# Alan-404/Conformer

Hardware: AMD Instinct MI355X
Metric: encoder audio-frames/sec (B=32,T=1000,d=512,L=16) (higher is better)
Workload: dtype f32; 1 GPU; cfg2 Conformer-L Encoder.forward: B=32/GPU, T=1000 mel frames (T'=249), d=512, 16 blocks, 8 heads, k=31, fp32, eval, random-init weights, batch-sharded replicas; per_gpu_batch=32, mel_frames=1000

## Files before the change

### conformer_amd/_lib.py

```python
from __future__ import annotations

import ctypes
import os
from ctypes import c_char_p, c_float, c_int, c_int64, c_uint64, c_void_p

_HERE = os.path.dirname(os.path.abspath(__file__))
LIB_PATH = os.environ.get("CONFORMER_AMD_LIB") or os.path.join(_HERE, "lib", "libconformer_hip.so")

_P, _I, _L, _F, _U = c_void_p, c_int, c_int64, c_float, c_uint64
ABI_VERSION = 4

SIGNATURES = {
    "cfm_version": (c_int, []),
    "cfm_abi_version": (c_int, []),
    "cfm_gemm_bias_stats_f32": (c_int, [_P, _P, _P, _P, _P, _L, _I, _I, _L, _L, _P]),
    "cfm_gemm_bias_residual_stats_f32": (c_int, [_P, _P, _P, _P, _F, _P, _P, _L, _I, _I, _L, _L, _L, _P]),
    "cfm_gemm_splitk_f32": (c_int, [_I, _P, _P, _P, _P, _F, _P, _P, _I, _L, _I, _I, _L, _L, _L, _P]),
    "cfm_gemm_lnfold_f32": (c_int, [_I, _P, _P, _I, _F, _P, _P, _P, _P, _L, _I, _I, _L, _L, _P]),
    "cfm_layernorm_fwd_stats_f32": (c_int, [_P, _P, _P, _P, _P, _L, _I, _F, _P]),
    "cfm_ffn_pack_elems": (ctypes.c_int64, [_I, _I]),
    "cfm_ffn_pack_f32": (c_int, [_P, _P, _P, _I, _I, _P]),
    "cfm_rowgemm_pack_f32": (c_int, [_P, _P, _I, _I, _I, _P]),
    "cfm_rowchain_f32": (c_int, [_I, _I, _I, _I, _P, _L, _P, _P, _P, _L, _P, _L, _P, _I, _F, _P, _P, _P, _P, _F, _I, _P, _L, _P, _P, _P, _F,
                                 _P, _P, _P, _F, _P, _L, _L, _I, _P]),
    "cfm_ffn_tile_stride_f4": (ctypes.c_int64, [_I]),
    "cfm_ffn_rotate": (c_int, []),
    "cfm_ffn_fused_f32": (c_int, [_P, _L, _P, _I, _F, _P, _P, _P, _P, _F, _P, _L, _I, _P, _P, _P, _F, _L, _I, _I, _P]),
    "cfm_strerror": (c_char_p, [_I]),
    "cfm_device_check": (c_int, []),
    "cfm_subsampled_length": (c_int64, [_L]),
    "cfm_subsampled_lengths_i64": (c_int, [_P, _P, _I, _P]),
    "cfm_layernorm_fwd_f32": (c_int, [_P, _P, _P, _P, _P, _P, _L, _I, _F, _P]),
    "cfm_gemm_bias_f32": (c_int, [_P, _P, _P, _P, _L, _I, _I, _L, _L, _P]),
    "cfm_gemm_bias_swish_f32": (c_int, [_P, _P, _P, _P, _L, _I, _I, _L, _L, _P]),
    "cfm_gemm_bias_relu_f32": (c_int, [_P, _P, _P, _P, _L, _I, _I, _L, _L, _P]),
    "cfm_gemm_bias_glu_f32": (c_int, [_P, _P, _P, _P, _L, _I, _I, _L, _L, _P]),
    "cfm_gemm_bias_residual_f32": (c_int, [_P, _P, _P, _P, _F, _P, _L, _I, _I, _L, _L, _L, _P]),
    "cfm_gemm_mfma16_f32": (c_int, [_I, _I, _P, _I, _P, _I, _P, _P, _F, _P, _I, _P, _I, _L, _I, _I, _L, _L, _L, _F, _U, _P]),
    "cfm_layernorm_fwd_out16_f32": (c_int, [_I, _P, _P, _P, _P, _P, _P, _L, _I, _F, _P]),
    "cfm_cast16_f32": (c_int, [_I, _P, _P, _L, _P]),
    "cfm_cast16_multi_f32": (c_int, [_I, _P, _I, _P]),
    "cfm_relpos_attention_mfma16_f32": (c_int, [_I, _P, _P, _P, _L, _P, _L, _P, _P, _P, _P, _L, _P, _I, _I, _I, _I, _F, _U, _P]),
    "cfm_relpos_attention_rows_mfma16_f32": (c_int, [_I, _P, _P, _P, _L, _P, _L, _P, _P, _P, _P, _L, _I, _I, _I, _I, _I, _I, _P]),
    "cfm_relpos_attention_io16_mfma16_f32": (c_int, [_I, _P, _P, _P, _I, _L, _P, _L, _P, _P, _P, _P, _I, _L, _I, _I, _I, _I, _P]),
    "cfm_subsample_conv2_relu_mfma16_f32": (c_int, [_I, _P, _I, _P, _I, _P, _P, _I, _I, _I, _I, _I, _P]),
    "cfm_subsample_conv1_relu_out16_f32": (c_int, [_I, _P, _P, _P, _P, _I, _I, _I, _I, _P]),
    "cfm_gemm_bwd_batched_mfma16_f32": (c_int, [_I, _P, _I, _L, _P, _I, _I, _L, _P, _I, _L, _F, _P, _L, _I, _I, _I, _L, _I, _I, _I, _I,
                                                _L, _L, _L, _L, _L, _L, _F, _U, _I, _P]),
    "cfm_subsample_conv2_bwd_weight_mfma16_f32": (c_int, [_I, _P, _P, _P, _I, _I, _I, _I, _P]),
    "cfm_subsample_conv2_bwd_input_mfma16_f32": (c_int, [_I, _P, _P, _P, _I, _I, _I, _I, _P]),
    "cfm_subsample_conv2_rowtab_elems": (ctypes.c_int64, [_I, _I, _I]),
    "cfm_subsample_conv2_bwd_weight_h16_mfma16_f32": (c_int, [_I, _P, _I, _P, _P, _P, _P, _I, _I, _I, _I, _P]),
    "cfm_relu_bwd_out16_f32": (c_int, [_I, _P, _P, _P, _L, _P]),
    "cfm_dwconv_bn_swish_fwd_out16_f32": (c_int, [_I, _P, _P, _P, _P, _P, _P, _P, _F, _P, _I, _I, _I, _I, _P]),
    "cfm_glu_bwd_out16_f32": (c_int, [_I, _P, _P, _P, _L, _I, _P]),
    "cfm_subsample_conv2_bwd_input_fwdkernel_mfma16_f32": (c_int, [_I, _P, _I, _P, _P, _P, _I, _I, _I, _I, _P]),
    "cfm_subsample_conv2_bwd_input_fwdkernel_out16_mfma16_f32": (c_int, [_I, _P, _I, _P, _P, _P, _I, _I, _I, _I, _P]),
    "cfm_subsample_conv1_bwd_d16_f32": (c_int, [_I, _P, _P, _P, _P, _P, _P, _I, _I, _I, _I, _P]),
    "cfm_reflect_pad_f32": (c_int, [_P, _P, _I, _L, _I, _L, _P]),
    "cfm_power_mel_log_f32": (c_int, [_P, _L, _P, _P, _I, _I, _I, _I, _F, _P]),
    "cfm_power_mel_log_mfma_f32": (c_int, [_P, _L, _P, _P, _I, _I, _I, _I, _I, _F, _P]),
    "cfm_dft_frames_f32": (c_int, [_P, _P, _P, _L, _I, _I, _I, _P]),
    "cfm_specaugment_apply_f32": (c_int, [_P, _I, _I, _I, _P, _I, _F, _P]),
    "cfm_gemm_bias_swish_save_f32": (c_int, [_P, _P, _P, _P, _P, _L, _I, _I, _L, _L, _P]),
    "cfm_gemm_bwd_f32": (c_int, [_P, _I, _L, _P, _I, _L, _P, _L, _F, _P, _L, _I, _I, _L, _I, _P]),
    "cfm_gemm_bwd_batched_f32": (c_int, [_P, _I, _L, _P, _I, _L, _P, _L, _F, _P, _L, _I, _I, _L, _I, _I, _I, _I,
                                         _L, _L, _L, _L, _L, _L, _F, _U, _P]),
    "cfm_gemm_train_f32": (c_int, [_I, _P, _P, _P, _P, _F, _P, _P, _L, _I, _I, _L, _L, _L, _F, _U, _P]),
    "cfm_relpos_attention_train_f32": (c_int, [_P, _P, _P, _L, _P, _L, _P, _P, _P, _P, _L, _P, _I, _I, _I, _I, _F, _U, _P]),
    "cfm_dropout_f32": (c_int, [_P, _P, _L, _F, _U, _P]),
    "cfm_dropout_out16_f32": (c_int, [_I, _P, _P, _L, _F, _U, _P]),
    "cfm_layernorm_bwd_dx_f32": (c_int, [_P, _P, _P, _P, _P, _P, _P, _L, _I, _P]),
    "cfm_layernorm_bwd_params_f32": (c_int, [_P, _P, _P, _P, _P, _P, _L, _I, _P]),
    "cfm_layernorm_bwd_f32": (c_int, [_P, _P, _P, _P, _P, _P, _P, _P, _P, _L, _I, _P, ctypes.c_size_t, _P]),
    "cfm_layernorm_bwd_workspace_bytes": (ctypes.c_size_t, [_L, _I]),
    "cfm_colsum_f32": (c_int, [_P, _L, _L, _I, _F, _P, _P]),
    "cfm_glu_fwd_f32": (c_int, [_P, _P, _L, _I, _P]),
    "cfm_glu_bwd_f32": (c_int, [_P, _P, _P, _L, _I, _P]),
    "cfm_dwconv_bn_swish_bwd_f32": (c_int, [_P, _P, _P, _P, _P, _P, _P, _P, _F, _I, _P, _P, _P, _P, _P, _P,
                                            _I, _I, _I, _I, _P]),
    "cfm_dwconv_bn_stats_workspace_bytes": (ctypes.c_size_t, [_I, _I, _I]),
    "cfm_dwconv_bn_stats_f32": (c_int, [_P, _P, _P, _P, _P, _P, _P, _F, _I, _I, _I, _I, _P, ctypes.c_size_t, _P]),
    "cfm_debug_attention_bwd_trace_f32": (c_int, [_P]),
    "cfm_debug_attention_bwd_trace_mfma16": (c_int, [_P]),
    "cfm_debug_gemm_mfma16_trace": (c_int, [_P]),
    "cfm_debug_gemm_mfma16_force_tile": (c_int, [_I]),
    "cfm_debug_gemm_last_tile": (c_int, [_I, _P]),
    "cfm_relpos_attention_bwd_mfma16_f32": (c_int, [_I, _P, _P, _P, _L, _P, _L, _P, _P, _P, _P, _P, _L, _P, _P, _P, _P, _L, _P, _L,
                                                    _P, _P, _I, _I, _I, _I, _F, _U, _P]),
    "cfm_relpos_attention_bwd_f32": (c_int, [_P, _P, _P, _L, _P, _L, _P, _P, _P, _P, _P, _L, _P, _P, _P, _P, _L, _P, _L, _P, _P,
                                             _I, _I, _I, _I, _F, _U, _I, _P]),
    "cfm_relu_bwd_f32": (c_int, [_P, _P, _P, _L, _P]),
    "cfm_subsample_conv2_bwd_weight_f32": (c_int, [_P, _P, _P, _I, _I, _I, _I, _P]),
    "cfm_pack_conv2_weight_t_f32": (c_int, [_P, _P, _I, _P]),
    "cfm_subsample_conv2_bwd_input_f32": (c_int, [_P, _P, _P, _I, _I, _I, _I, _P]),
    "cfm_subsample_conv1_bwd_f32": (c_int, [_P, _P, _P, _P, _P, _P, _I, _I, _I, _I, _P]),
    "cfm_adam_step_f32": (c_int, [_P, _I, _F, _F, _F, _F, _F, _F, _P]),
    "cfm_greedy_ctc_decode_f32": (c_int, [_P, _P, _P, _P, _P, _I, _I, _I, _I, _I, _P]),
    "cfm_ctc_beam_workspace_bytes": (ctypes.c_size_t, [_I, _I, _I, _I]),
    "cfm_ctc_beam_decode_f32": (c_int, [_P, _P, _I, _I, _I, _I, _I, _I, _F, _F, _I, _P, ctypes.c_size_t, _P, _P, _P, _P, _P]),
    "cfm_ngram_lm_pack_bytes": (ctypes.c_size_t, [_I, _P, _I, _L, _I, _L]),
    "cfm_ngram_lm_pack": (c_int, [_I, _P, _P, _P, _P, _I, _P, _P, _I, _I, _I, _I, _P, _P, _P, _P, ctypes.c_size_t]),
    "cfm_ngram_lm_score_f64": (c_int, [_P, _P, _P, _I, _I, _P, _P]),
    "cfm_ctc_beam_lm_workspace_bytes": (ctypes.c_size_t, [_I, _I, _I, _I]),
    "cfm_ctc_beam_lm_decode_f32": (c_int, [_P, _P, _I, _I, _I, _I, _I, _I, _F, _F, _I, _P, ctypes.c_double, ctypes.c_double,
                                           ctypes.c_double, _I, _P, ctypes.c_size_t, _P, _P, _P, _P, _P, _P]),
    "cfm_hotword_pack_bytes": (ctypes.c_size_t, [_I, _L, _I, _L, _I, _L]),
    "cfm_hotword_pack": (c_int, [_I, _P, _P, _I, _P, _P, _I, _P, _P, _P, _P, ctypes.c_size_t]),
    "cfm_hotword_count": (c_int, [_P, _P, _P, _I, ctypes.c_double, _P, _P, _P]),
    "cfm_ctc_beam_hw_workspace_bytes": (ctypes.c_size_t, [_I, _I, _I, _I]),
    "cfm_ctc_beam_hw_decode_f32": (c_int, [_P, _P, _I, _I, _I, _I, _I, _I, _F, _F, _I, _P, ctypes.c_double, ctypes.c_double,
                                           ctypes.c_double, _I, _P, ctypes.c_double, _P, ctypes.c_size_t, _P, _P, _P, _P, _P,
                                           _P]),
    "cfm_ctc_beam_stream_state_bytes": (ctypes.c_size_t, [_I, _I, _I, _I, _I, _I]),
    "cfm_ctc_beam_stream_init": (c_int, [_I, _I, _I, _I, _P, _I, _P, _P, ctypes.c_size_t, _P]),
    "cfm_ctc_beam_stream_step_f32": (c_int, [_P, _P, _I, _I, _I, _I, _I, _I, _F, _F, _I, _P, ctypes.c_double, ctypes.c_double,
                                             ctypes.c_double, _I, _P, ctypes.c_double, _P, ctypes.c_size_t, _I, _I, _P, _P, _P,
                                             _P, _P, _P]),
    "cfm_ctc_beam_stream_finish_f32": (c_int, [_I, _I, _I, _I, _P, ctypes.c_double, ctypes.c_double, ctypes.c_double, _I, _P,
                                               ctypes.c_double, _P, ctypes.c_size_t, _I, _P, _P, _P, _P, _P, _P]),
    "cfm_ctc_beam_stream_reset_slots": (c_int, [_I, _I, _I, _I, _P, _I, _P, _P, _I, _P, ctypes.c_size_t, _P]),
    "cfm_lstm_fwd_carry_f32": (c_int, [_P, _P, _P, _P, _P, _P, _P, _P, _I, _I, _I, _P]),
    "cfm_lstm_fwd_frag_carry_f32": (c_int, [_P, _P, _P, _P, _P, _P, _P, _P, _P, _I, _I, _I, _P]),
    "cfm_lstm_fwd_mfma16_carry_f32": (c_int, [_I, _P, _P, _P, _P, _P, _P, _P, _P, _P, _I, _I, _I, _P]),
    "cfm_lstm_fwd_f32": (c_int, [_P, _P, _P, _P, _P, _P, _P, _I, _I, _I, _P]),
    "cfm_lstm_fwd_frag_f32": (c_int, [_P, _P, _P, _P, _P, _P, _P, _P, _I, _I, _I, _P]),
    "cfm_lstm_bwd_frag_f32": (c_int, [_P, _P, _P, _P, _P, _P, _P, _P, _I, _I, _I, _P]),
    "cfm_debug_lstm_trace": (c_int, [_P]),
    "cfm_debug_dw16_trace": (c_int, [_P]),
    "cfm_linear_bwd_weight_mfma16_f32": (c_int, [_I, _P, _I, _L, _P, _I, _L, _P, _L, _P, _I, _I, _L, _F, _P]),
    "cfm_lstm_fwd_mfma16_f32": (c_int, [_I, _P, _P, _P, _P, _P, _P, _P, _P, _I, _I, _I, _P]),
    "cfm_lstm_bwd_mfma16_f32": (c_int, [_I, _P, _P, _P, _P, _P, _P, _P, _P, _I, _I, _I, _P]),
    "cfm_lstm_bwd_f32": (c_int, [_P, _P, _P, _P, _P, _P, _P, _I, _I, _I, _P]),
    "cfm_swish_bn_eval_f32": (c_int, [_P, _P, _P, _P, _P, _F, _P, _L, _I, _P]),
    "cfm_swish_bn_stats_f32": (c_int, [_P, _P, _P, _P, _P, _F, _L, _I, _P]),
    "cfm_swish_bn_bwd_f32": (c_int, [_P, _P, _P, _P, _P, _F, _I, _P, _P, _P, _L, _I, _P]),
    "cfm_split_pack_elems": (ctypes.c_int64, [_I, _I, _I]),
    "cfm_split_pack_bf16_f32": (c_int, [_I, _P, _P, _I, _I, _P]),
    "cfm_gemm_split_bf16_f32": (c_int, [_I, _I, _P, _P, _P, _P, _F, _P, _L, _I, _I, _L, _L, _L, _P]),
    "cfm_subsample_conv2_relu_split_bf16_f32": (c_int, [_I, _P, _P, _P, _P, _I, _I, _I, _I, _P]),
    "cfm_ctc_workspace_floats": (ctypes.c_int64, [_I, _I, _I]),
    "cfm_ctc_loss_fwd_f32": (c_int, [_P, _P, _P, _L, _L, _P, _P, _I, _I, _I, _I, _I, _P, _P, _P]),
    "cfm_ctc_loss_bwd_f32": (c_int, [_P, _P, _P, _L, _L, _P, _P, _I, _I, _I, _I, _I, _P, _P, _P, _P]),
    "cfm_ctc_align_workspace_bytes": (ctypes.c_size_t, [_I, _I, _I]),
    "cfm_ctc_align_f32": (c_int, [_P, _P, _P, _P, _I, _I, _I, _I, _I, _P, ctypes.c_size_t, _P, _P, _P, _P, _P, _P, _P, _P]),
    "cfm_relpos_attention_rows_f32": (c_int, [_P, _P, _P, _L, _P, _L, _P, _P, _P, _P, _L, _I, _I, _I, _I, _I, _I, _I, _P, _P]),
    "cfm_relpos_attention_slots_f32": (c_int, [_P, _P, _P, _L, _P, _L, _P, _P, _P, _P, _P, _P, _L, _I, _I, _I, _I, _I, _I, _P, _P]),
    "cfm_relpos_attention_slots_mfma16_f32": (c_int, [_I, _P, _P, _P, _I, _L, _P, _L, _P, _P, _P, _P, _P, _P, _L, _I, _I, _I, _I, _I, _I,
                                                      _P, _P]),
    "cfm_debug_attention_trace_f32": (c_int, [_P, _P, _P, _L, _P, _L, _P, _P, _P, _P, _L, _I, _I, _I, _I, _P, _P]),
    "cfm_debug_set_bwd_tile": (c_int, [_I]),
    "cfm_debug_set_attention_waves": (c_int, [_I]),
    "cfm_debug_gemm_cfg_f32": (c_int, [_I, _P, _P, _P, _P, _F, _P, _L, _I, _I, _P, _P]),
    "cfm_debug_set_conv2_bk": (c_int, [_I]),
    "cfm_debug_ffn_trace": (c_int, [_P, _I]),
    "cfm_debug_ffn_variant": (c_int, [_I]),
    "cfm_debug_ffn_layout": (c_int, [_I, _I]),
    "cfm_relpos_table_f32": (c_int, [_P, _P, _I, _I, _P]),
    "cfm_relpos_attention_fwd_f32": (c_int, [_P, _P, _P, _L, _P, _L, _P, _P, _P, _P, _L, _P, _I, _I, _I, _I, _P]),
    "cfm_dwconv_bn_swish_fwd_f32": (c_int, [_P, _P, _P, _P, _P, _P, _P, _F, _P, _I, _I, _I, _I, _P]),
    "cfm_convmod_glu_dwconv_f32": (c_int, [_P, _L, _P, _I, _F, _P, _P, _P, _P, _P, _P, _P, _P, _P, _F, _P, _L, _I, _I, _I, _I, _P]),
    "cfm_debug_convmod_variant": (c_int, [_I]),
    "cfm_subsample_conv1_relu_f32": (c_int, [_P, _P, _P, _P, _I, _I, _I, _I, _P]),
    "cfm_pack_conv2_weight_f32": (c_int, [_P, _P, _I, _P]),
    "cfm_subsample_conv2_relu_f32": (c_int, [_P, _P, _P, _P, _I, _I, _I, _I, _P]),
    "cfm_pack_linear_weight_f32": (c_int, [_P, _P, _I, _I, _I, _P]),
    "cfm_conv2_wino_plane_elems": (c_int64, [_I, _I, _I, _I]),
    "cfm_pack_conv2_wino_weight_f32": (c_int, [_P, _P, _I, _P]),
    "cfm_subsample_conv2_wino_relu_f32": (c_int, [_P, _P, _P, _P, _P, _I, _I, _I, _I, _P]),
}


class ConformerHipError(RuntimeError):
    pass


_lib = None


def load() -> ctypes.CDLL:
    global _lib
    if _lib is not None:
        return _lib
    if not os.path.exists(LIB_PATH):
        raise ConformerHipError(
            f"{LIB_PATH} is missing: build it with `python -m conformer_amd.build` "
            "(there is no CPU/eager fallback for the Conformer hot path)")
    import torch
    lib = ctypes.CDLL(LIB_PATH, mode=ctypes.RTLD_GLOBAL)
    try:
        lib.cfm_abi_version.restype = c_int
        got = int(lib.cfm_abi_version())
    except AttributeError:
        got = 0
    if got != ABI_VERSION:
        raise ConformerHipError(f"{LIB_PATH} implements C-ABI revision {got}, this binding needs {ABI_VERSION}: rebuild it with "
                                "`python -m conformer_amd.build`")
    for name, (res, args) in SIGNATURES.items():
        fn = getattr(lib, name)
        fn.restype = res
        fn.argtypes = args
    _lib = lib
    return lib


class CastItem(ctypes.Structure):
    _fields_ = [("src", ctypes.c_void_p), ("dst", ctypes.c_void_p), ("rows", ctypes.c_int64), ("cols", ctypes.c_int64),
                ("transpose", ctypes.c_int)]


CALLS = [0]


def check(status: int, what: str) -> None:
    CALLS[0] += 1
    if status != 0:
        msg = load().cfm_strerror(status).decode()
        raise ConformerHipError(f"{what} failed: {msg} (status {status})")
```

### conformer_amd/csrc/rowchain_f32.hip

```cpp
#include <type_traits>

#include "cfm_common.h"

namespace {

struct ChainArgs {
    const float* X; int64_t ldx;
    const float* Wpre; const float* bpre; const float* R; int64_t ldr; float* Y1; int64_t ldy1;
    const float* ln_stats; int ln_parts;
    float ln_eps;
    const float* Wp; const float* b1f; const float* cs1; const float* b2; float alpha; int hidden; int64_t tile_stride; int rotate;
    float* Y; int64_t ldy; float* stats_out; const float* gamma2; const float* beta2; float eps2;
    const float* Wpost; const float* bpost; const float* cspost; float post_eps; float* Z; int64_t ldz;
    int64_t M;
};

enum { CH_PLAIN = 0, CH_STATS = 1, CH_LN = 2 };
enum { POST_NONE = 0, POST_BIAS3 = 1, POST_GLU = 2 };

template <int ND, int PRE, int CORE, int POST, int MODE>
__global__ __launch_bounds__(256, 1) void rowchain_f32_kernel(const ChainArgs a) {
    constexpr int D = 32 * ND, XS = D + 4, NL = 4 * ND, RING = 16;
    constexpr int TPW = ND / 4, QW = 32 * TPW, EW = QW + 4, ERS = 32 * EW;
    static_assert(NL % RING == 0 && ND % 4 == 0, "d = 128, 256 or 512");
    static_assert(CORE || (PRE && POST), "a chain without the feed-forward is PRE + POST");
    __shared__ __attribute__((aligned(16))) float smem[32 * XS + 4 * ERS + 64];
    float* Xs = smem;
    float* Ys = smem + 32 * XS;
    float* St = Ys + 4 * ERS;

    const int tid = threadIdx.x, lane = tid & 63, li = lane & 31, hf = lane >> 5;
    const int wave = __builtin_amdgcn_readfirstlane(tid >> 6);
    const int64_t m0 = (int64_t)blockIdx.x * 32;
    constexpr int V = D / 4;

    f32x16 y[ND];
    const float* xrow = Xs + li * XS + 4 * hf;
    float mean = 0.f, rstd = 0.f;

    auto gemm_rows = [&](const f32x4* ws, auto nt_tag) {
        constexpr int NT = decltype(nt_tag)::value;
        constexpr int CB = NT > 12 ? 1 : NT > 4 ? 2 : NT > 2 ? 4 : NT > 1 ? 8 : 16, RS = CB * NT;
        static_assert(NL % CB == 0, "");
#pragma unroll
        for (int t = 0; t < NT; ++t)
#pragma unroll
            for (int r = 0; r < 16; ++r) y[t][r] = 0.f;
        f32x4 rg[RS];
#pragma unroll
        for (int i = 0; i < RS; ++i) rg[i] = ws[i * 64];
        constexpr int TOTAL = NL * NT;
        f32x4 xv = *reinterpret_cast<const f32x4*>(xrow);
#pragma unroll 1
        for (int c0 = 0; c0 < NL; c0 += CB) {
            const f32x4* wn = ws + (int64_t)min((c0 + CB) * NT, TOTAL - RS) * 64;
            const float* xc = xrow + 8 * c0;
#pragma unroll
            for (int cc = 0; cc < CB; ++cc) {
                const f32x4 xn = *reinterpret_cast<const f32x4*>(xc + 8 * (cc + 1));
#pragma unroll
                for (int t = 0; t < NT; t += (NT % 2 == 0 ? 2 : 1)) {
                    const int i = cc * NT + t;
                    if constexpr (NT % 2 == 0) {
                        const f32x4 w0 = rg[i], w1 = rg[i + 1];
                        rg[i] = wn[i * 64];
                        rg[i + 1] = wn[(i + 1) * 64];
#pragma unroll
                        for (int e = 0; e < 4; ++e) {
                            y[t] = __builtin_amdgcn_mfma_f32_32x32x2f32(w0[e], xv[e], y[t], 0, 0, 0);
                            y[t + 1] = __builtin_amdgcn_mfma_f32_32x32x2f32(w1[e], xv[e], y[t + 1], 0, 0, 0);
                        }
                    } else {
                        const f32x4 w0 = rg[i];
                        rg[i] = wn[i * 64];
#pragma unroll
                        for (int e = 0; e < 4; ++e) y[t] = __builtin_amdgcn_mfma_f32_32x32x2f32(w0[e], xv[e], y[t], 0, 0, 0);
                    }
                    __builtin_amdgcn_sched_barrier(0);
                }
                xv = xn;
            }
        }
    };
    auto row_stats = [&](float eps, float* store_to, int64_t ld) {
#pragma unroll 2
        for (int rr = 0; rr < 8; ++rr) {
            const int r = 8 * wave + rr;
            f32x4 v[(V + 63) / 64];
            float s = 0.f;
#pragma unroll
            for (int i = 0; i < (V + 63) / 64; ++i) {
                const int c4 = lane + 64 * i;
                v[i] = c4 < V ? *reinterpret_cast<const f32x4*>(Xs + r * XS + 4 * c4) : f32x4{0.f, 0.f, 0.f, 0.f};
                s += (v[i][0] + v[i][1]) + (v[i][2] + v[i][3]);
                if (store_to && c4 < V && m0 + r < a.M) *reinterpret_cast<f32x4*>(store_to + (m0 + r) * ld + 4 * c4) = v[i];
            }
            const float mu = wave_sum(s) * (1.0f / (float)D);
            float q = 0.f;
#pragma unroll
            for (int i = 0; i < (V + 63) / 64; ++i) {
                if (lane + 64 * i < V) {
                    const f32x4 dv = v[i] - mu;
                    q += (dv[0] * dv[0] + dv[1] * dv[1]) + (dv[2] * dv[2] + dv[3] * dv[3]);
                }
            }
            q = wave_sum(q);
            if (lane == 0) { St[2 * r] = mu; St[2 * r + 1] = 1.0f / sqrtf(q * (1.0f / (float)D) + eps); }
        }
        __syncthreads();
        mean = St[2 * li]; rstd = St[2 * li + 1];
    };

    {
#pragma unroll
        for (int p = 0; p < 32 * V / 256; ++p) {
            const int f = tid + 256 * p, r = f / V, c4 = f % V;
            const int64_t row = min(m0 + r, a.M - 1);
            *reinterpret_cast<f32x4*>(Xs + r * XS + 4 * c4) = *reinterpret_cast<const f32x4*>(a.X + row * a.ldx + 4 * c4);
            if constexpr (PRE) *reinterpret_cast<f32x4*>(Ys + r * XS + 4 * c4) = *reinterpret_cast<const f32x4*>(a.R + row * a.ldr + 4 * c4);
        }
    }
    if constexpr (!PRE) {
        const float* sp = a.ln_stats + min(m0 + li, a.M - 1) * a.ln_parts * 2;
        const float ni = (float)(D / a.ln_parts), inv_ni = 1.0f / ni;
        float cnt = 0.f, mu = 0.f, m2 = 0.f;
        for (int p = 0; p < a.ln_parts; ++p) {
            const float2 sq = *reinterpret_cast<const float2*>(sp + 2 * p);
            const float dl = sq.x * inv_ni - mu, tot = cnt + ni;
            mu += dl * (ni / tot);
            m2 += sq.y + dl * dl * (cnt * ni / tot);
            cnt = tot;
        }
        mean = mu;
        rstd = 1.0f / sqrtf(m2 * (1.0f / (float)D) + a.ln_eps);
    }
    __syncthreads();

    if constexpr (PRE) {
        gemm_rows(reinterpret_cast<const f32x4*>(a.Wpre) + (int64_t)wave * NL * TPW * 64 + lane, std::integral_constant<int, TPW>{});
        __syncthreads();
#pragma unroll
        for (int t = 0; t < TPW; ++t)
#pragma unroll
            for (int q = 0; q < 4; ++q) {
                const int col = QW * wave + 32 * t + 8 * q + 4 * hf;
                const f32x4 bb = *reinterpret_cast<const f32x4*>(a.bpre + col);
                const f32x4 rr = *reinterpret_cast<const f32x4*>(Ys + li * XS + col);
                *reinterpret_cast<f32x4*>(Xs + li * XS + col) =
                    f32x4{y[t][4 * q], y[t][4 * q + 1], y[t][4 * q + 2], y[t][4 * q + 3]} + bb + rr;
            }
        __syncthreads();
        row_stats(a.ln_eps, a.Y1, a.ldy1);
    }

    if constexpr (CORE) {
        const int NS = a.hidden >> 7;
        const f32x4* wp = reinterpret_cast<const f32x4*>(a.Wp) + lane;
        const int64_t TILE = a.tile_stride;
        const int rot = a.rotate ? (int)((blockIdx.x >> 3) % (unsigned)NS) : 0;
        f32x4 ring[RING];
        {
            const f32x4* sb = wp + (4 * rot + wave) * TILE;
#pragma unroll
            for (int i = 0; i < RING; ++i) ring[i] = sb[i * 64];
        }
#pragma unroll
        for (int t = 0; t < ND; ++t)
#pragma unroll
            for (int r = 0; r < 16; ++r) y[t][r] = 0.f;
        for (int s = 0; s < NS; ++s) {
            const int sr = s + rot < NS ? s + rot : s + rot - NS;
            const int g = 4 * sr + wave;
            const f32x4* sb = wp + g * TILE;
            const f32x4* nb = wp + (4 * (sr + 1 < NS ? sr + 1 : 0) + wave) * TILE;
            f32x4 csv[4], b1v[4];
#pragma unroll
            for (int q = 0; q < 4; ++q) {
                csv[q] = *reinterpret_cast<const f32x4*>(a.cs1 + g * 32 + 8 * q + 4 * hf);
                b1v[q] = *reinterpret_cast<const f32x4*>(a.b1f + g * 32 + 8 * q + 4 * hf);
            }
            f32x16 ha;
#pragma unroll
            for (int r = 0; r < 16; ++r) ha[r] = 0.f;
            f32x4 xv = *reinterpret_cast<const f32x4*>(xrow);
#pragma unroll
            for (int c = 0; c < NL; ++c) {
                const f32x4 xn = *reinterpret_cast<const f32x4*>(xrow + 8 * (c + 1));
                const f32x4 wv = ring[c % RING];
                ring[c % RING] = sb[(c + RING) * 64];
                ha = __builtin_amdgcn_mfma_f32_32x32x2f32(wv[0], xv[0], ha, 0, 0, 0);
                ha = __builtin_amdgcn_mfma_f32_32x32x2f32(wv[1], xv[1], ha, 0, 0, 0);
                ha = __builtin_amdgcn_mfma_f32_32x32x2f32(wv[2], xv[2], ha, 0, 0, 0);
                ha = __builtin_amdgcn_mfma_f32_32x32x2f32(wv[3], xv[3], ha, 0, 0, 0);
                xv = xn;
                __builtin_amdgcn_sched_barrier(0);
            }
            float sw[16];
#pragma unroll
            for (int r = 0; r < 16; ++r) {
                const float v = rstd * (ha[r] - mean * csv[r >> 2][r & 3]) + b1v[r >> 2][r & 3];
                sw[r] = swishf_acc(v);
            }
#pragma unroll
            for (int j = 0; j < NL; j += 2) {
                const int q = j / ND, t = j % ND;
                const f32x4 w0 = ring[j % RING], w1 = ring[(j + 1) % RING];
                ring[j % RING] = j + RING < NL ? sb[(NL + j + RING) * 64] : nb[(j + RING - NL) * 64];
                ring[(j + 1) % RING] = j + 1 + RING < NL ? sb[(NL + j + 1 + RING) * 64] : nb[(j + 1 + RING - NL) * 64];
#pragma unroll
                for (int e = 0; e < 4; ++e) {
                    y[t] = __builtin_amdgcn_mfma_f32_32x32x2f32(w0[e], sw[4 * q + e], y[t], 0, 0, 0);
                    y[t + 1] = __builtin_amdgcn_mfma_f32_32x32x2f32(w1[e], sw[4 * q + e], y[t + 1], 0, 0, 0);
                }
                __builtin_amdgcn_sched_barrier(0);
            }
        }

        float* Ex = Ys;
        const bool cok = 4 * li < QW;
        const int cl = cok ? 4 * li : 0;
        f32x4 v[4][4];
#pragma unroll
        for (int c = 0; c < 4; ++c) {
#pragma unroll
            for (int k = 0; k < TPW; ++k)
#pragma unroll
                for (int q = 0; q < 4; ++q)
                    *reinterpret_cast<f32x4*>(Ex + wave * ERS + li * EW + 32 * k + 8 * q + 4 * hf) =
                        f32x4{y[c * TPW + k][4 * q], y[c * TPW + k][4 * q + 1], y[c * TPW + k][4 * q + 2], y[c * TPW + k][4 * q + 3]};
            const f32x4 b2v = *reinterpret_cast<const f32x4*>(a.b2 + QW * c + cl);
            __syncthreads();
#pragma unroll
            for (int it = 0; it < 4; ++it) {
                const int r = 8 * wave + 2 * it + hf;
                const float* e = Ex + r * EW + cl;
                f32x4 acc = *reinterpret_cast<const f32x4*>(e);
                acc += *reinterpret_cast<const f32x4*>(e + ERS);
                acc += *reinterpret_cast<const f32x4*>(e + 2 * ERS);
                acc += *reinterpret_cast<const f32x4*>(e + 3 * ERS);
                const f32x4 xr = *reinterpret_cast<const f32x4*>(Xs + r * XS + QW * c + cl);
                v[c][it] = cok ? a.alpha * (acc + b2v) + xr : f32x4{0.f, 0.f, 0.f, 0.f};
            }
            __syncthreads();
        }
        auto half_sum = [](float (&t)[4]) {
#pragma unroll
            for (int o = 16; o > 0; o >>= 1)
#pragma unroll
                for (int it = 0; it < 4; ++it) t[it] += __shfl_xor(t[it], o, 64);
        };
        if constexpr (POST) {
            float s[4], q[4];
#pragma unroll
            for (int it = 0; it < 4; ++it) {
                s[it] = 0.f;
#pragma unroll
                for (int c = 0; c < 4; ++c) {
                    s[it] += (v[c][it][0] + v[c][it][1]) + (v[c][it][2] + v[c][it][3]);
                    if (cok) *reinterpret_cast<f32x4*>(Xs + (8 * wave + 2 * it + hf) * XS + QW * c + cl) = v[c][it];
                }
            }
            half_sum(s);
#pragma unroll
            for (int it = 0; it < 4; ++it) {
                const float mu = s[it] * (1.0f / (float)D);
                q[it] = 0.f;
#pragma unroll
                for (int c = 0; c < 4; ++c) {
                    if (cok) {
                        const f32x4 dv = v[c][it] - mu;
                        q[it] += (dv[0] * dv[0] + dv[1] * dv[1]) + (dv[2] * dv[2] + dv[3] * dv[3]);
                    }
                }
                s[it] = mu;
            }
            half_sum(q);
#pragma unroll
            for (int it = 0; it < 4; ++it)
                if (li == 0) {
                    St[2 * (8 * wave + 2 * it + hf)] = s[it];
                    St[2 * (8 * wave + 2 * it + hf) + 1] = 1.0f / sqrtf(q[it] * (1.0f / (float)D) + a.post_eps);
                }
        }
        if constexpr (MODE == CH_LN) {
            f32x4 gam[4], bet[4];
#pragma unroll
            for (int c = 0; c < 4; ++c) {
                gam[c] = *reinterpret_cast<const f32x4*>(a.gamma2 + QW * c + cl);
                bet[c] = *reinterpret_cast<const f32x4*>(a.beta2 + QW * c + cl);
            }
            float s[4], q[4];
#pragma unroll
            for (int it = 0; it < 4; ++it) {
                s[it] = 0.f;
#pragma unroll
                for (int c = 0; c < 4; ++c) s[it] += (v[c][it][0] + v[c][it][1]) + (v[c][it][2] + v[c][it][3]);
            }
            half_sum(s);
#pragma unroll
            for (int it = 0; it < 4; ++it) {
                const float mu = s[it] * (1.0f / (float)D);
                q[it] = 0.f;
#pragma unroll
                for (int c = 0; c < 4; ++c) {
                    if (cok) {
                        v[c][it] = v[c][it] - mu;
                        q[it] += (v[c][it][0] * v[c][it][0] + v[c][it][1] * v[c][it][1]) + (v[c][it][2] * v[c][it][2] + v[c][it][3] * v[c][it][3]);
                    }
                }
            }
            half_sum(q);
#pragma unroll
            for (int it = 0; it < 4; ++it) {
                const float rs = 1.0f / sqrtf(q[it] * (1.0f / (float)D) + a.eps2);
                s[it] = 0.f;
#pragma unroll
                for (int c = 0; c < 4; ++c) {
                    if (cok) {
                        v[c][it] = v[c][it] * rs * gam[c] + bet[c];
                        s[it] += (v[c][it][0] + v[c][it][1]) + (v[c][it][2] + v[c][it][3]);
                    }
                }
            }
            if (a.stats_out) {
                half_sum(s);
#pragma unroll
                for (int it = 0; it < 4; ++it) {
                    const float mo = s[it] * (1.0f / (float)D);
                    q[it] = 0.f;
#pragma unroll
                    for (int c = 0; c < 4; ++c) {
                        if (cok) {
                            const f32x4 tt = v[c][it] - mo;
                            q[it] += (tt[0] * tt[0] + tt[1] * tt[1]) + (tt[2] * tt[2] + tt[3] * tt[3]);
                        }
                    }
                }
                half_sum(q);
#pragma unroll
                for (int it = 0; it < 4; ++it) {
                    const int64_t row = m0 + 8 * wave + 2 * it + hf;
                    if (li == 0 && row < a.M) *reinterpret_cast<float2*>(a.stats_out + 2 * row) = float2{s[it], q[it]};
                }
            }
        }
#pragma unroll
        for (int it = 0; it < 4; ++it) {
            const int64_t row = m0 + 8 * wave + 2 * it + hf;
            const bool row_ok = row < a.M;
#pragma unroll
            for (int c = 0; c < 4; ++c) {
                if (row_ok && cok) *reinterpret_cast<f32x4*>(a.Y + row * a.ldy + QW * c + cl) = v[c][it];
                if constexpr (MODE == CH_STATS) {
                    float s = (v[c][it][0] + v[c][it][1]) + (v[c][it][2] + v[c][it][3]);
                    s += __shfl_xor(s, 1, 64); s += __shfl_xor(s, 2, 64); s += __shfl_xor(s, 4, 64);
                    const float m = s * (1.0f / 32.0f);
                    const f32x4 dv = v[c][it] - m;
                    float q = (dv[0] * dv[0] + dv[1] * dv[1]) + (dv[2] * dv[2] + dv[3] * dv[3]);
                    q += __shfl_xor(q, 1, 64); q += __shfl_xor(q, 2, 64); q += __shfl_xor(q, 4, 64);
                    if (row_ok && cok && (li & 7) == 0)
                        *reinterpret_cast<float2*>(a.stats_out + (row * (int64_t)ND + ((QW * c + cl) >> 5)) * 2) = float2{s, q};
                }
            }
        }
        if constexpr (POST) {
            __syncthreads();
            mean = St[2 * li]; rstd = St[2 * li + 1];
        }
    }

    if constexpr (POST != POST_NONE) {
        constexpr int NT = POST == POST_BIAS3 ? 3 * TPW : 2 * TPW;
        constexpr int NOUT = POST == POST_BIAS3 ? 3 * D : D;
        gemm_rows(reinterpret_cast<const f32x4*>(a.Wpost) + (int64_t)wave * NL * NT * 64 + lane, std::integral_constant<int, NT>{});
        float* stg = Ys + wave * ERS;
        const bool cok = 4 * li < QW;
        const int cl = cok ? 4 * li : 0;
        constexpr int NP = POST == POST_BIAS3 ? 3 : 1;
#pragma unroll
        for (int p = 0; p < NP; ++p) {
#pragma unroll
            for (int k = 0; k < TPW; ++k)
#pragma unroll
                for (int q = 0; q < 4; ++q) {
                    f32x4 o;
                    if constexpr (POST == POST_GLU) {
                        const int n = QW * wave + 32 * k + 8 * q + 4 * hf;
                        const f32x4 cv = *reinterpret_cast<const f32x4*>(a.cspost + n), cg = *reinterpret_cast<const f32x4*>(a.cspost + D + n);
                        const f32x4 bv = *reinterpret_cast<const f32x4*>(a.bpost + n), bg = *reinterpret_cast<const f32x4*>(a.bpost + D + n);
#pragma unroll
                        for (int e = 0; e < 4; ++e) {
                            const float val = rstd * (y[k][4 * q + e] - mean * cv[e]) + bv[e];
                            const float gat = rstd * (y[TPW + k][4 * q + e] - mean * cg[e]) + bg[e];
                            o[e] = val * sigmoidf_acc(gat);
                        }
                    } else {
                        const int n = 32 * NT * wave + 32 * (TPW * p + k) + 8 * q + 4 * hf;
                        const f32x4 cv = *reinterpret_cast<const f32x4*>(a.cspost + n);
                        const f32x4 bv = *reinterpret_cast<const f32x4*>(a.bpost + n);
#pragma unroll
                        for (int e = 0; e < 4; ++e) o[e] = rstd * (y[TPW * p + k][4 * q + e] - mean * cv[e]) + bv[e];
                    }
                    *reinterpret_cast<f32x4*>(stg + li * EW + 32 * k + 8 * q + 4 * hf) = o;
                }
            __builtin_amdgcn_fence(__ATOMIC_RELEASE, "wavefront");
            __builtin_amdgcn_wave_barrier();
            __builtin_amdgcn_fence(__ATOMIC_ACQUIRE, "wavefront");
            const int colbase = POST == POST_GLU ? QW * wave : 32 * NT * wave + QW * p;
#pragma unroll
            for (int it = 0; it < 16; ++it) {
                const int r = 2 * it + hf;
                const f32x4 o = *reinterpret_cast<const f32x4*>(stg + r * EW + cl);
                if (cok && m0 + r < a.M) *reinterpret_cast<f32x4*>(a.Z + (m0 + r) * a.ldz + colbase + cl) = o;
            }
            __builtin_amdgcn_fence(__ATOMIC_RELEASE, "wavefront");
            __builtin_amdgcn_wave_barrier();
        }
        (void)NOUT;
    }
}

__global__ __launch_bounds__(256) void rowgemm_pack_kernel(const float* __restrict__ W, float* __restrict__ Wp, int N, int d, int glu) {
    const int nl = d >> 3, nt = N >> 7, tpw = d >> 7;
    const int64_t total = (int64_t)4 * nl * nt * 64;
    for (int64_t f = (int64_t)blockIdx.x * 256 + threadIdx.x; f < total; f += (int64_t)gridDim.x * 256) {
        const int lane = (int)(f & 63), li = lane & 31, hf = lane >> 5;
        int64_t r = f >> 6;
        const int t = (int)(r % nt); r /= nt;
        const int c = (int)(r % nl), w = (int)(r / nl);
        const int row = glu ? (t < tpw ? 32 * (tpw * w + t) : d + 32 * (tpw * w + t - tpw)) : 32 * (nt * w + t);
        reinterpret_cast<f32x4*>(Wp)[f] = *reinterpret_cast<const f32x4*>(W + (int64_t)(row + li) * d + 8 * c + 4 * hf);
    }
}

}

extern "C" int cfm_rowgemm_pack_f32(const float* W, float* Wp, int N, int d, int glu, cfm_stream_t stream) {
    CFM_REQUIRE(W && Wp, CFM_ERR_NULL);
    CFM_REQUIRE((d == 128 || d == 256 || d == 512) && N > 0 && N % 128 == 0 && (!glu || N == 2 * d), CFM_ERR_UNSUPPORTED);
    CFM_REQUIRE(CFM_ALIGNED16(W) && CFM_ALIGNED16(Wp), CFM_ERR_ALIGN);
    const int64_t total = (int64_t)N * d / 4;
    const unsigned blocks = (unsigned)((total + 255) / 256 < 4096 ? (total + 255) / 256 : 4096);
    hipLaunchKernelGGL(rowgemm_pack_kernel, dim3(blocks), dim3(256), 0, static_cast<hipStream_t>(stream), W, Wp, N, d, glu);
    return cfm_launch_status();
}

extern "C" int64_t cfm_ffn_tile_stride_f4(int d);
extern "C" int cfm_ffn_rotate(void);

extern "C" int cfm_rowchain_f32(int pre, int core, int post, int mode, const float* X, int64_t ldx, const float* Wpre_packed,
                                const float* bpre, const float* R, int64_t ldr, float* Y1, int64_t ldy1, const float* ln_stats,
                                int ln_parts, float ln_eps, const float* Wffn_packed, const float* b1f, const float* colsum1,
                                const float* b2, float alpha, int hidden, float* Y, int64_t ldy, float* stats_out,
                                const float* gamma2, const float* beta2, float eps2, const float* Wpost_packed, const float* bpost,
                                const float* cspost, float post_eps, float* Z, int64_t ldz, int64_t M, int d, cfm_stream_t stream) {
    CFM_REQUIRE(X && M >= 0 && ldx >= d && ldx % 4 == 0 && CFM_ALIGNED16(X), CFM_ERR_BAD_SHAPE);
    CFM_REQUIRE(d == 128 || d == 256 || d == 512, CFM_ERR_UNSUPPORTED);
    CFM_REQUIRE((pre == 0 || pre == 1) && (core == 0 || core == 1) && post >= 0 && post <= 2 && mode >= 0 && mode <= 2, CFM_ERR_UNSUPPORTED);
    CFM_REQUIRE(core || (pre && post), CFM_ERR_UNSUPPORTED);
    if (pre) {
        CFM_REQUIRE(Wpre_packed && bpre && R, CFM_ERR_NULL);
        CFM_REQUIRE(ldr >= d && ldr % 4 == 0 && CFM_ALIGNED16(Wpre_packed) && CFM_ALIGNED16(bpre) && CFM_ALIGNED16(R), CFM_ERR_ALIGN);
        CFM_REQUIRE(!Y1 || (ldy1 >= d && ldy1 % 4 == 0 && CFM_ALIGNED16(Y1)), CFM_ERR_ALIGN);
    } else {
        CFM_REQUIRE(ln_stats, CFM_ERR_NULL);
        CFM_REQUIRE(ln_parts >= 1 && ln_parts <= 16 && (ln_parts & (ln_parts - 1)) == 0 && (reinterpret_cast<uintptr_t>(ln_stats) & 7u) == 0,
                    CFM_ERR_UNSUPPORTED);
    }
    if (core) {
        CFM_REQUIRE(Wffn_packed && b1f && colsum1 && b2 && Y, CFM_ERR_NULL);
        CFM_REQUIRE(hidden > 0 && hidden % 128 == 0, CFM_ERR_UNSUPPORTED);
        CFM_REQUIRE(ldy >= d && ldy % 4 == 0 && CFM_ALIGNED16(Wffn_packed) && CFM_ALIGNED16(b1f) && CFM_ALIGNED16(colsum1) && CFM_ALIGNED16(b2) &&
                    CFM_ALIGNED16(Y) && (reinterpret_cast<uintptr_t>(stats_out) & 7u) == 0, CFM_ERR_ALIGN);
        CFM_REQUIRE(mode != CH_STATS || stats_out, CFM_ERR_NULL);
        CFM_REQUIRE(mode != CH_LN || (gamma2 && beta2 && CFM_ALIGNED16(gamma2) && CFM_ALIGNED16(beta2)), CFM_ERR_NULL);
    }
    if (post) {
        const int nout = post == POST_BIAS3 ? 3 * d : d;
        CFM_REQUIRE(Wpost_packed && bpost && cspost && Z, CFM_ERR_NULL);
        CFM_REQUIRE(ldz >= nout && ldz % 4 == 0 && CFM_ALIGNED16(Wpost_packed) && CFM_ALIGNED16(bpost) && CFM_ALIGNED16(cspost) && CFM_ALIGNED16(Z),
                    CFM_ERR_ALIGN);
    }
    if (M == 0) return CFM_OK;
    ChainArgs a{X, ldx, Wpre_packed, bpre, R, ldr, Y1, ldy1, ln_stats, ln_parts, ln_eps, Wffn_packed, b1f, colsum1, b2, alpha, hidden,
                cfm_ffn_tile_stride_f4(d), cfm_ffn_rotate(), Y, ldy, stats_out, gamma2, beta2, eps2, Wpost_packed, bpost, cspost,
                post_eps, Z, ldz, M};
    const dim3 grid((unsigned)((M + 31) / 32)), block(256);
    hipStream_t s = static_cast<hipStream_t>(stream);
#define CH_LAUNCH(ND, PRE, CORE, POST, MODE) hipLaunchKernelGGL((rowchain_f32_kernel<ND, PRE, CORE, POST, MODE>), grid, block, 0, s, a)
#define CH_BY_D(PRE, CORE, POST, MODE) do { if (d == 512) CH_LAUNCH(16, PRE, CORE, POST, MODE); else if (d == 256) CH_LAUNCH(8, PRE, CORE, POST, MODE); \
                                            else CH_LAUNCH(4, PRE, CORE, POST, MODE); } while (0)
    if (!pre && core && post == POST_BIAS3 && mode == CH_PLAIN) CH_BY_D(0, 1, POST_BIAS3, CH_PLAIN);
    else if (pre && !core && post == POST_GLU) CH_BY_D(1, 0, POST_GLU, CH_PLAIN);
    else if (pre && core && post == POST_NONE && mode == CH_LN) CH_BY_D(1, 1, POST_NONE, CH_LN);
    else return CFM_ERR_UNSUPPORTED;
#undef CH_BY_D
#undef CH_LAUNCH
    return cfm_launch_status();
}
```

### conformer_amd/model/modules/encoder.py

```python
from typing import Optional, Tuple

import torch
import torch.nn as nn

from ... import autograd as ag
from ... import ops
from ..utils._guard import STRICT, PackCache, active_dropout, refuse_dropout
from ..utils.block import ConformerBlock
from ..utils.convolution import ConvolutionSubsampling
from ..utils.position import RelativePositionalEncoding


class Encoder(nn.Module):
    def __init__(self, n_mel_channels: int, n_blocks: int, d_model: int, n_heads: int, kernel_size: int,
                 dropout_rate: float = 0.0) -> None:
        super().__init__()
        self.n_freq_out = ((n_mel_channels - 1) // 2 - 1) // 2
        self.downsampling_conv = ConvolutionSubsampling(channels=d_model)
        self.linear = nn.Linear(in_features=d_model * self.n_freq_out, out_features=d_model)
        self.dropout = nn.Dropout(p=dropout_rate)
        self.rel_pe = RelativePositionalEncoding(d_model=d_model)
        self.layers = nn.ModuleList([ConformerBlock(d_model=d_model, n_heads=n_heads, kernel_size=kernel_size,
                                                    dropout_rate=dropout_rate) for _ in range(n_blocks)])
        self._packs = PackCache()
        self.cache_projected_positions = False

    def forward(self, x: torch.Tensor, lengths: Optional[torch.Tensor] = None) -> Tuple[torch.Tensor, Optional[torch.Tensor]]:
        refuse_dropout(self, "Encoder")
        d = self.linear.out_features
        h = self.downsampling_conv.channel_last(x)
        st = None
        out_len = ConvolutionSubsampling.out_lengths(lengths)
        if ag.needs_grad(self.linear):
            wlp = self.linear.weight.view(d, d, self.n_freq_out).transpose(1, 2).reshape(d, -1)
            h = ag.LinearFn.apply(h, wlp, self.linear.bias, active_dropout(self.dropout))
        else:
            wlp = self._packs.get("wlp", (self.linear.weight,),
                                  lambda: ops.pack_linear_weight(self.linear.weight, d, self.n_freq_out))
            fold = ops.ln_fold_ok(d) and len(self.layers) > 0 and h.dtype == torch.float32 and self.layers[0]._ln_fold(h)
            if fold:
                h, st = ops.linear(h, wlp, self.linear.bias, emit_stats=True)
            else:
                h = ops.linear(h, wlp, self.linear.bias)
        n_frames = h.shape[1]
        if out_len is not None:
            if out_len.device != h.device:
                out_len = out_len.to(h.device)
            if STRICT and int(out_len.max()) != n_frames:
                raise RuntimeError(f"lengths.max() after subsampling must equal T'={n_frames}")
        table = self.rel_pe.table(n_frames)
        pos_all = self._projected_positions(table)
        for i, layer in enumerate(self.layers):
            h, st = layer.fused_chain(h, table, out_len, None if pos_all is None else pos_all[:, i * d:(i + 1) * d],
                                      x_stats=st, want_stats=i + 1 < len(self.layers))
        return h, out_len

    def _projected_positions(self, table: torch.Tensor) -> Optional[torch.Tensor]:
        if len(self.layers) == 0:
            return None
        ws = [l.attention.attention.pos_proj.weight for l in self.layers]
        bs = [l.attention.attention.pos_proj.bias for l in self.layers]

        if ag.needs_grad(self.layers):
            return ag.LinearFn.apply(table, torch.cat(ws, dim=0), torch.cat(bs, dim=0))
        w = self._packs.get("pos_w", ws, lambda: torch.cat([t.detach() for t in ws], dim=0).contiguous())
        b = self._packs.get("pos_b", bs, lambda: torch.cat([t.detach() for t in bs], dim=0).contiguous())
        if self.cache_projected_positions:
            return self._packs.get("pos_all", (w, b, table), lambda: ops.linear(table, w, b))
        return ops.linear(table, w, b)
```

### conformer_amd/model/utils/block.py

```python
from typing import Optional

import torch
import torch.nn as nn

from ... import autograd as ag
from ... import ops
from .attention import MultiHeadSelfAttentionModule
from .convolution import ConvolutionModule
from .ffn import FeedForwardModule
from ._guard import refuse_dropout
from .masking import lengths_from_key_padding_mask


class ConformerBlock(nn.Module):
    def __init__(self, d_model: int, n_heads: int, kernel_size: int, dropout_rate: float = 0.0) -> None:
        super().__init__()
        self.ffn_1 = FeedForwardModule(dim=d_model, dropout_rate=dropout_rate)
        self.attention = MultiHeadSelfAttentionModule(n_heads=n_heads, d_model=d_model, dropout_rate=dropout_rate)
        self.conv = ConvolutionModule(channels=d_model, kernel_size=kernel_size, dropout_rate=dropout_rate)
        self.ffn_2 = FeedForwardModule(dim=d_model, dropout_rate=dropout_rate)
        self.layer_norm = nn.LayerNorm(normalized_shape=d_model)

    def fused(self, x: torch.Tensor, pos_table: torch.Tensor, lengths: Optional[torch.Tensor],
              pos_projected: Optional[torch.Tensor] = None) -> torch.Tensor:
        return self.fused_chain(x, pos_table, lengths, pos_projected)[0]

    def _ln_fold(self, x: torch.Tensor) -> bool:
        bn = self.conv.batch_norm
        return (x.dtype == torch.float32 and ops.ln_fold_ok(self.layer_norm.normalized_shape[0])
                and not (bn.training or bn.running_mean is None) and not ag.needs_grad(self, x))

    def fused_chain(self, x: torch.Tensor, pos_table: torch.Tensor, lengths: Optional[torch.Tensor],
                    pos_projected: Optional[torch.Tensor] = None, x_stats: Optional[torch.Tensor] = None,
                    want_stats: bool = False, stream=None):
        if stream is not None:
            bn = self.conv.batch_norm
            if bn.training or bn.running_mean is None or ag.needs_grad(self, x):
                raise RuntimeError("ConformerBlock.fused_chain: a stream context is for inference only (eval-mode BatchNorm "
                                   "under torch.no_grad())")
        if not self._ln_fold(x):
            y = self.ffn_1.fused(x, residual=x, alpha=0.5)
            y = self.attention.fused(y, pos_table, lengths, residual=y, pos_projected=pos_projected, stream=stream)
            y = self.conv.fused(y, residual=y, stream=stream)
            y = self.ffn_2.fused(y, residual=y, alpha=0.5)
            if ag.needs_grad(self.layer_norm, y):
                return ag.LayerNormFn.apply(y, self.layer_norm.weight, self.layer_norm.bias, self.layer_norm.eps), None
            return ops.layernorm(y, self.layer_norm.weight, self.layer_norm.bias, self.layer_norm.eps), None
        if stream is None and x_stats is not None and x.is_contiguous() and ops.rowchain_ok(
                x.shape[-1], self.ffn_1.hidden_linear.out_features, x.numel() // x.shape[-1]):
            return self._row_chains(x, pos_table, lengths, pos_projected, x_stats, want_stats)
        y, st = self.ffn_1.fused(x, residual=x, alpha=0.5, stats=x_stats, emit_stats=True)
        y, st = self.attention.fused(y, pos_table, lengths, residual=y, pos_projected=pos_projected, stats=st, emit_stats=True,
                                      stream=stream)
        y, st = self.conv.fused(y, residual=y, stats=st, emit_stats=True, stream=stream)
        ln = self.layer_norm
        if stream is None and self.ffn_2.fuses(y, y, st):
            if want_stats:
                return self.ffn_2.fused(y, residual=y, alpha=0.5, stats=st, emit_stats=True, closing_ln=ln)
            return self.ffn_2.fused(y, residual=y, alpha=0.5, stats=st, closing_ln=ln), None
        y = self.ffn_2.fused(y, residual=y, alpha=0.5, stats=st)
        if want_stats:
            return ops.layernorm(y, ln.weight, ln.bias, ln.eps, emit_stats=True)
        return ops.layernorm(y, ln.weight, ln.bias, ln.eps), None

    def _row_chains(self, x, pos_table, lengths, pos_projected, x_stats, want_stats):
        f1, f2, att, cv = self.ffn_1, self.ffn_2, self.attention, self.conv
        a, ln_a, ln_c = att.attention, att.layer_norm, cv.layer_norm
        for m, name in ((f1, "FeedForwardModule"), (att, "MultiHeadSelfAttentionModule"), (a, "RelativeMultiHeadAttention"),
                        (cv, "ConvolutionModule"), (f2, "FeedForwardModule")):
            refuse_dropout(m, name)
        ffn1 = f1._packs.get("ffn_pack", (f1.hidden_linear.weight, f1.hidden_linear.bias, f1.layer_norm.weight, f1.layer_norm.bias,
                                          f1.out_linear.weight), f1._pack)
        ffn2 = f2._packs.get("ffn_pack", (f2.hidden_linear.weight, f2.hidden_linear.bias, f2.layer_norm.weight, f2.layer_norm.bias,
                                          f2.out_linear.weight), f2._pack)
        wqkv, bqkv = a._qkv_params()

        def fold_pack(w, b, ln, glu=False):
            wf, bf, cs = ops.fold_layernorm(w, b, ln.weight, ln.bias)
            return ops.rowgemm_pack(wf, glu=glu), bf, cs

        wq_p, bq_f, csq = a._packs.get("qkv_chain", (wqkv, bqkv, ln_a.weight, ln_a.bias), lambda: fold_pack(wqkv, bqkv, ln_a))
        wo_p = a._packs.get("out_chain", (a.out_proj.weight,), lambda: ops.rowgemm_pack(a.out_proj.weight.detach()))
        pw1, pw2 = cv.pointwise_conv_1, cv.pointwise_conv_2
        wg_p, bg_f, csg = cv._packs.get("pw1_chain", (pw1.weight, pw1.bias, ln_c.weight, ln_c.bias),
                                        lambda: fold_pack(pw1.weight, pw1.bias, ln_c, glu=True))
        w2_p = cv._packs.get("pw2_chain", (pw2.weight,), lambda: ops.rowgemm_pack(pw2.weight.detach()))
        y, qkv = ops.rowchain_ffn_qkv(x, x_stats, ffn1, f1.out_linear.bias, 0.5, f1.layer_norm.eps, wq_p, bq_f, csq, ln_a.eps)
        pos = pos_projected if pos_projected is not None else ops.linear(pos_table, a.pos_proj.weight, a.pos_proj.bias)
        ctx = ops.relpos_attention(qkv, pos, a.content_bias, a.position_bias, lengths, a.n_heads)
        y2, g = ops.rowchain_out_glu(ctx, wo_p, a.out_proj.bias, y, wg_p, bg_f, csg, ln_c.eps)
        c = cv.depthwise_eval(g)
        ln = self.layer_norm
        return ops.rowchain_pw2_ffn_ln(c, w2_p, pw2.bias, y2, ffn2, f2.out_linear.bias, 0.5, f2.layer_norm.eps,
                                       (ln.weight, ln.bias, ln.eps), want_stats)

    def forward(self, x: torch.Tensor, pos_embedding: torch.Tensor, mask: Optional[torch.Tensor] = None) -> torch.Tensor:
        table = pos_embedding[0] if pos_embedding.dim() == 3 else pos_embedding
        lengths = None if mask is None else lengths_from_key_padding_mask(mask)
        return self.fused(x, table, lengths)
```

### conformer_amd/model/utils/convolution.py

```python
from typing import Optional, Tuple

import torch
import torch.nn as nn
import torch.nn.functional as F

from ... import autograd as ag
from ... import ops
from ._guard import PackCache, active_dropout, refuse_dropout
from .activation import GLU, Swish


class ConvolutionModule(nn.Module):
    def __init__(self, channels: int, kernel_size: int, dropout_rate: float = 0.0) -> None:
        super().__init__()
        self.layer_norm = nn.LayerNorm(normalized_shape=channels)
        self.pointwise_conv_1 = nn.Conv1d(channels, channels * 2, kernel_size=1)
        self.glu = GLU(dim=1)
        self.deepwise_conv = nn.Conv1d(channels, channels, kernel_size=kernel_size, padding=(kernel_size - 1) // 2,
                                       groups=channels)
        self.batch_norm = nn.BatchNorm1d(num_features=channels)
        self.swish = Swish()
        self.pointwise_conv_2 = nn.Conv1d(channels, channels, kernel_size=1)
        self.dropout = nn.Dropout(p=dropout_rate)
        self._packs = PackCache()

    def depthwise_eval(self, g: torch.Tensor, for_gemm: bool = False) -> torch.Tensor:
        bn = self.batch_norm
        return ops.dwconv_bn_swish(g, self.deepwise_conv.weight, self.deepwise_conv.bias, bn.weight, bn.bias,
                                   bn.running_mean, bn.running_var, bn.eps, for_gemm=for_gemm)

    def fused(self, x: torch.Tensor, residual: Optional[torch.Tensor] = None, stats: Optional[torch.Tensor] = None,
              emit_stats: bool = False, stream=None):
        refuse_dropout(self, "ConvolutionModule")
        bn = self.batch_norm
        train_bn = bn.training or bn.running_mean is None
        if train_bn and (bn.momentum is None or not bn.track_running_stats):
            raise NotImplementedError("ConvolutionModule: only the default BatchNorm1d(momentum=0.1, "
                                      "track_running_stats=True) is built")
        if train_bn and not ag.needs_grad(self, x, residual):
            h = ops.layernorm(x, self.layer_norm.weight, self.layer_norm.bias, self.layer_norm.eps, for_gemm=True)
            g = ops.linear_glu(h, self.pointwise_conv_1.weight, self.pointwise_conv_1.bias)
            bm, bv = ops.dwconv_bn_batch_stats(g, self.deepwise_conv.weight, self.deepwise_conv.bias, bn.running_mean,
                                               bn.running_var, bn.momentum)
            bn.num_batches_tracked += 1
            s = ops.dwconv_bn_swish(g, self.deepwise_conv.weight, self.deepwise_conv.bias, bn.weight, bn.bias, bm, bv,
                                    bn.eps, for_gemm=True)
            if residual is None:
                return ops.linear(s, self.pointwise_conv_2.weight, self.pointwise_conv_2.bias)
            return ops.linear_residual(s, self.pointwise_conv_2.weight, self.pointwise_conv_2.bias, residual, 1.0)
        if ag.needs_grad(self, x, residual):
            if residual is not None and residual is not x:
                raise NotImplementedError("ConvolutionModule.fused: pass residual=x (block.py:23)")
            out = ag.ConvModuleFn.apply(x, self.layer_norm.weight, self.layer_norm.bias, self.pointwise_conv_1.weight,
                                        self.pointwise_conv_1.bias, self.deepwise_conv.weight, self.deepwise_conv.bias,
                                        bn.weight, bn.bias, bn.running_mean, bn.running_var,
                                        self.pointwise_conv_2.weight, self.pointwise_conv_2.bias,
                                        self.layer_norm.eps, bn.eps, train_bn, bn.momentum if train_bn else 0.0,
                                        active_dropout(self.dropout))
            if train_bn:
                bn.num_batches_tracked += 1
            return out if residual is not None else out - x
        if stats is not None:
            ln, pw1 = self.layer_norm, self.pointwise_conv_1
            wf, bf, cs = self._packs.get("ln_fold", (pw1.weight, pw1.bias, ln.weight, ln.bias),
                                         lambda: ops.fold_layernorm(pw1.weight, pw1.bias, ln.weight, ln.bias))
            dw = self.deepwise_conv
            if stream is None and x.dim() == 3 and ops.convmod_fused_ok(x.shape[0], x.shape[1], x.shape[2], dw.weight.shape[-1]):
                g = None
                s = ops.convmod_glu_dwconv(x, stats, wf, bf, cs, ln.eps, dw.weight, dw.bias, bn.weight, bn.bias, bn.running_mean,
                                           bn.running_var, bn.eps)
            else:
                g = ops.linear_lnfold(x, stats, wf, bf, cs, ln.eps, glu=True)
        else:
            h = ops.layernorm(x, self.layer_norm.weight, self.layer_norm.bias, self.layer_norm.eps, for_gemm=stream is None)
            g = ops.linear_glu(h, self.pointwise_conv_1.weight, self.pointwise_conv_1.bias)
        if g is not None:
            s = self.depthwise_eval(g, for_gemm=True) if stream is None else stream.depthwise(self, g)
        if residual is None:
            if emit_stats:
                return ops.linear(s, self.pointwise_conv_2.weight, self.pointwise_conv_2.bias, emit_stats=True)
            return ops.linear(s, self.pointwise_conv_2.weight, self.pointwise_conv_2.bias)
        return ops.linear_residual(s, self.pointwise_conv_2.weight, self.pointwise_conv_2.bias, residual, 1.0, emit_stats=emit_stats)

    def forward(self, x: torch.Tensor) -> torch.Tensor:
        return self.fused(x)


class ConvolutionSubsampling(nn.Module):
    def __init__(self, channels: int) -> None:
        super().__init__()
        self.conv_1 = nn.Conv2d(1, channels, kernel_size=3, stride=2)
        self.act_1 = nn.ReLU()
        self.conv_2 = nn.Conv2d(channels, channels, kernel_size=3, stride=2)
        self.act_2 = nn.ReLU()
        self._packs = PackCache()

    @staticmethod
    def out_lengths(lengths: Optional[torch.Tensor]) -> Optional[torch.Tensor]:
        if lengths is None:
            return None
        if lengths.is_cuda and lengths.dtype == torch.int64:
            return ops.subsampled_lengths(lengths)
        return torch.div(torch.div(lengths - 1, 2, rounding_mode="floor") - 1, 2, rounding_mode="floor")

    def channel_last(self, x: torch.Tensor) -> torch.Tensor:
        if ag.needs_grad(self, x):
            if x.requires_grad:
                raise NotImplementedError("ConvolutionSubsampling: the gradient w.r.t. the input spectrogram is not "
                                          "built (the reference never needs it: the input is data)")
            return ag.SubsampleStemFn.apply(x, self.conv_1.weight, self.conv_1.bias, self.conv_2.weight, self.conv_2.bias)
        w2p = self._packs.get("w2p", (self.conv_2.weight,), lambda: ops.pack_conv2_weight(self.conv_2.weight))
        w2w = None
        if ops.conv2_winograd_ok(self.conv_2.weight.shape[0]):
            w2w = self._packs.get("w2w", (self.conv_2.weight,), lambda: ops.pack_conv2_wino_weight(self.conv_2.weight))
        return ops.subsample_stem(x, self.conv_1.weight, self.conv_1.bias, w2p, self.conv_2.bias, w2w=w2w)

    def forward(self, x: torch.Tensor, lengths: Optional[torch.Tensor] = None) -> Tuple[torch.Tensor, Optional[torch.Tensor]]:
        h = self.channel_last(x)
        if h.dtype != torch.float32:
            h = h.float()
        B, T2, _ = h.shape
        C = self.conv_1.out_channels
        h = h.view(B, T2, -1, C).transpose(2, 3).reshape(B, T2, -1)
        return h, self.out_lengths(lengths)


class DepthWiseSeperableConvolution(nn.Module):

    def __init__(self, in_channels: int, out_channels: int) -> None:
        super().__init__()
        self.depth_wise_conv = nn.Conv2d(in_channels, out_channels, kernel_size=3, stride=2, groups=in_channels)
        self.point_wise_conv = nn.Conv2d(out_channels, out_channels, kernel_size=1)

    def forward(self, x: torch.Tensor):
        return self.point_wise_conv(self.depth_wise_conv(x))


class DownsamplingConvolution(nn.Module):

    def __init__(self, channels: int) -> None:
        super().__init__()
        self.conv_1 = DepthWiseSeperableConvolution(1, channels)
        self.conv_2 = DepthWiseSeperableConvolution(channels, channels)

    def forward(self, x: torch.Tensor, lengths: Optional[torch.Tensor]):
        h = F.relu(self.conv_2(F.relu(self.conv_1(x.unsqueeze(1)))))
        B, C, Fp, Tp = h.shape
        h = h.permute(0, 3, 1, 2).reshape(B, Tp, C * Fp)
        return h, ConvolutionSubsampling.out_lengths(lengths)
```

### conformer_amd/ops.py

```python
from __future__ import annotations

import threading
import ctypes
from typing import Optional, Tuple

import torch

from . import _lib
from ._derived import DerivedCache


def _stream() -> int:
    return torch.cuda.current_stream().cuda_stream


def _req(t: torch.Tensor, name: str, dtype=torch.float32) -> torch.Tensor:
    if not isinstance(t, torch.Tensor) or not t.is_cuda:
        raise _lib.ConformerHipError(
            f"{name}: expected a tensor on a HIP device, got {getattr(t, 'device', type(t))}; "
            "the Conformer hot path only exists as gfx950 kernels (no CPU fallback)")
    if t.dtype != dtype:
        raise _lib.ConformerHipError(f"{name}: expected dtype {dtype}, got {t.dtype}")
    return t if t.is_contiguous() else t.contiguous()

# ... 29 lines not shown

    def __init__(self, prec: int) -> None:
        self.prec, self.prev = prec, None

    def __enter__(self):
        self.prev = getattr(_tls, "forced", None)
        _tls.forced = self.prec
        return self

    def __exit__(self, *exc):
        _tls.forced = self.prev
        return False


def bf16_mfma_active() -> bool:
    return mfma16_prec() == PREC_BF16


_WEIGHT_COPIES = DerivedCache()
def weight16(w: torch.Tensor, prec: int, transposed: bool = False) -> Optional[torch.Tensor]:
    if w.shape[-1] % 8 or w.numel() % 4 or (transposed and w.shape[0] % 8):
        return None
    def make() -> torch.Tensor:
        if transposed:
            out = torch.empty(w.shape[1], w.shape[0], device=w.device, dtype=_DT16[prec])
            item = (_lib.CastItem * 1)()
            item[0].src, item[0].dst, item[0].rows, item[0].cols, item[0].transpose = w.data_ptr(), out.data_ptr(), w.shape[0], w.shape[1], 1
            _lib.check(_lib.load().cfm_cast16_multi_f32(prec, ctypes.addressof(item), 1, _stream()), "cfm_cast16_multi_f32")
        else:
            out = torch.empty(w.shape, device=w.device, dtype=_DT16[prec])
            _lib.check(_lib.load().cfm_cast16_f32(prec, w.data_ptr(), out.data_ptr(), w.numel(), _stream()), "cfm_cast16_f32")
        return out
    return _WEIGHT_COPIES.get((w.data_ptr(), transposed), (w,), make, extra=prec)


def refresh_weight16(params) -> int:
    by_prec = {}
    def queue(p, transposed, prec, shape2, out) -> bool:
        ok = len(shape2) == 2 and shape2[0] * shape2[1] == p.numel() and p.is_contiguous()
        if ok:
            by_prec.setdefault(prec, []).append((p.detach().reshape(shape2), out, transposed))
        return ok
    for p in params:
        for t in (False, True):
            _WEIGHT_COPIES.refresh((p.data_ptr(), t), (p,), lambda prec, shapes, out: queue(p, t, prec, shapes[0], out))
    n = 0
    for prec, items in by_prec.items():
        arr = (_lib.CastItem * len(items))()
        for i, (w2, out, transposed) in enumerate(items):
            arr[i].src, arr[i].dst = w2.data_ptr(), out.data_ptr()
            arr[i].rows, arr[i].cols, arr[i].transpose = w2.shape[0], w2.shape[1], int(transposed)
        _lib.check(_lib.load().cfm_cast16_multi_f32(prec, ctypes.addressof(arr), len(items), _stream()), "cfm_cast16_multi_f32")
        n += len(items)
    return n


_ZERO_BIAS = {}


def _zero_bias(n: int, device) -> torch.Tensor:
    t = _ZERO_BIAS.get((n, device))
    if t is None:
        t = _ZERO_BIAS[(n, device)] = torch.zeros(n, device=device, dtype=torch.float32)
    return t


_FP32_MATMUL = {"native": 0, "bf16x6": 3, "bf16x3": 2}
_fp32_planes = _FP32_MATMUL[__import__("os").environ.get("CONFORMER_AMD_FP32_MATMUL", "native")]


def set_fp32_matmul(mode: str) -> str:
    global _fp32_planes
    if mode not in _FP32_MATMUL:
        raise ValueError(f"fp32 matmul mode must be one of {sorted(_FP32_MATMUL)}, got {mode!r}")
    prev = fp32_matmul()
    _fp32_planes = _FP32_MATMUL[mode]
    return prev


def fp32_matmul() -> str:
    return {v: k for k, v in _FP32_MATMUL.items()}[_fp32_planes]


def weight_split(w: torch.Tensor, planes: int) -> Optional[torch.Tensor]:
    if w.dim() != 2 or w.shape[1] % 16:
        return None
    def make() -> torch.Tensor:
        lib = _lib.load()
        n, k = w.shape
        out = torch.empty(int(lib.cfm_split_pack_elems(planes, n, k)), device=w.device, dtype=torch.bfloat16)
        _lib.check(lib.cfm_split_pack_bf16_f32(planes, w.data_ptr(), out.data_ptr(), n, k, _stream()), "cfm_split_pack_bf16_f32")
        return out
    return _WEIGHT_COPIES.get((w.data_ptr(), "split"), (w,), make, extra=planes)


def unpack_weight_split(packed: torch.Tensor, planes: int, n: int, k: int) -> torch.Tensor:
    nb, ks = (n + 31) // 32, k // 16
    p = packed.view(nb, ks, planes, 2, 32, 8)
    return p.permute(2, 0, 4, 1, 3, 5).reshape(planes, nb * 32, k)[:, :n]


def _split_gemm(epi: int, a, w2, b, c, m, n, k, res=None, alpha: float = 1.0):
    if not _fp32_planes or a.dtype != torch.float32 or c.dtype != torch.float32:
        return None
    ws = weight_split(w2, _fp32_planes) if (epi != 3 or n % 32 == 0) else None
    if ws is None:
        return None
    _lib.check(_lib.load().cfm_gemm_split_bf16_f32(_fp32_planes, epi, a.data_ptr(), ws.data_ptr(), b.data_ptr(), _p(res), alpha,
                                                   c.data_ptr(), m, n, k, k, n, n, _stream()), "cfm_gemm_split_bf16_f32")
    return c


def out16_ok(k: int) -> int:
    prec = mfma16_prec()
    return prec if prec and k % 8 == 0 else 0


def _mfma16_gemm(prec: int, epi: int, a, w2, b, c, m, n, k, res=None, alpha: float = 1.0, z=None, drop_p: float = 0.0,
                 seed: int = 0):
    w16 = weight16(w2, prec)
    a16 = a.dtype != torch.float32
    if a16 and (w16 is None or a.dtype != _DT16[prec]):
        raise _lib.ConformerHipError(f"16-bit A operand ({a.dtype}) does not match the precision mode / weight shape")
    st = _lib.load().cfm_gemm_mfma16_f32(prec, epi, a.data_ptr(), int(a16), (w2 if w16 is None else w16).data_ptr(),
                                         int(w16 is not None), b.data_ptr(), _p(res), alpha, c.data_ptr(),
                                         int(c.dtype != torch.float32), _p(z), int(z is not None and z.dtype != torch.float32),
                                         m, n, k, k, n, n, float(drop_p), int(seed), _stream())
    _lib.check(st, "cfm_gemm_mfma16_f32")
    return c


def subsampled_length(n: int) -> int:
    return int(_lib.load().cfm_subsampled_length(int(n)))


def subsampled_lengths(lengths: torch.Tensor) -> torch.Tensor:
    lengths = _req(lengths, "lengths", torch.int64)
    out = torch.empty(lengths.shape, device=lengths.device, dtype=torch.int64)
    if lengths.numel():
        _lib.check(_lib.load().cfm_subsampled_lengths_i64(lengths.data_ptr(), out.data_ptr(), lengths.numel(), _stream()),
                   "cfm_subsampled_lengths_i64")
    return out


_LN_FOLD = __import__("os").environ.get("CONFORMER_AMD_LN_FOLD", "1") != "0"


def set_ln_fold(on: bool) -> bool:
    global _LN_FOLD
    prev, _LN_FOLD = _LN_FOLD, bool(on)
    return prev


def ln_fold_ok(d: int) -> bool:
    return bool(_LN_FOLD and not _fp32_planes and mfma16_prec() == PREC_F32 and d in (32, 64, 128, 256, 512))


def fold_layernorm(w: torch.Tensor, b: torch.Tensor, gamma: torch.Tensor, beta: torch.Tensor):
    w2 = w.detach().reshape(w.shape[0], -1)
    wf = (w2 * gamma.detach()[None, :]).contiguous()
    bf = (b.detach().double() + w2.double() @ beta.detach().double()).float().contiguous()
    cs = wf.double().sum(dim=1).float().contiguous()
    return wf, bf, cs


def linear_lnfold(a, stats, wf, bf, cs, eps: float, act: str = "none", glu: bool = False) -> torch.Tensor:
    a = _req(a, "A"); wf = _req(wf, "Wf"); bf = _req(bf, "bias_f"); cs = _req(cs, "colsum"); stats = _req(stats, "ln_stats")
    k = a.shape[-1]
    m = a.numel() // k
    n = wf.shape[0] // 2 if glu else wf.shape[0]
    if wf.shape[1] != k or stats.dim() != 3 or stats.shape[0] != m or stats.shape[2] != 2:
        raise _lib.ConformerHipError(f"linear_lnfold: A(...,{k}), Wf{tuple(wf.shape)}, stats{tuple(stats.shape)} do not match")
    c = torch.empty(*a.shape[:-1], n, device=a.device, dtype=torch.float32)
    epi = 3 if glu else {"none": 0, "swish": 1}[act]
    _lib.check(_lib.load().cfm_gemm_lnfold_f32(epi, a.data_ptr(), stats.data_ptr(), stats.shape[1], float(eps), wf.data_ptr(),
                                               bf.data_ptr(), cs.data_ptr(), c.data_ptr(), m, n, k, k, n, _stream()),
               "cfm_gemm_lnfold_f32")
    return c


_FFN_FUSED = __import__("os").environ.get("CONFORMER_AMD_FFN_FUSED", "1") != "0"


def set_ffn_fused(on: bool) -> bool:
    global _FFN_FUSED
    prev, _FFN_FUSED = _FFN_FUSED, bool(on)
    return prev


def ffn_fused_ok(d: int, hidden: int, rows: int) -> bool:
    if not (_FFN_FUSED and ln_fold_ok(d) and d in (128, 256, 512) and hidden % 128 == 0):
        return False
    blocks = (rows + 31) // 32
    rounds = (blocks + 255) // 256
    return blocks >= 0.9 * 256 * rounds


_FFN_LAYOUT_ENV = __import__("os").environ.get("CONFORMER_AMD_FFN_ROTATE")


def ffn_pack(w1f: torch.Tensor, w2: torch.Tensor) -> torch.Tensor:
    w1f = _req(w1f, "W1f"); w2 = _req(w2, "W2")
    hidden, d = w1f.shape
    if tuple(w2.shape) != (d, hidden):
        raise _lib.ConformerHipError(f"ffn_pack: W1f{tuple(w1f.shape)} and W2{tuple(w2.shape)} do not match")
    lib = _lib.load()
    if _FFN_LAYOUT_ENV is not None:
        lib.cfm_debug_ffn_layout(-1, int(_FFN_LAYOUT_ENV))
    wp = torch.zeros(int(lib.cfm_ffn_pack_elems(d, hidden)), device=w1f.device, dtype=torch.float32)
    _lib.check(lib.cfm_ffn_pack_f32(w1f.data_ptr(), w2.data_ptr(), wp.data_ptr(), d, hidden, _stream()), "cfm_ffn_pack_f32")
    return wp


def ffn_fused(x: torch.Tensor, stats: torch.Tensor, wp: torch.Tensor, b1f: torch.Tensor, cs: torch.Tensor, b2: torch.Tensor,
              alpha: float, eps: float, emit_stats: bool = False, closing_ln=None):
    x = _req(x, "x"); stats = _req(stats, "ln_stats"); wp = _req(wp, "Wp"); b1f = _req(b1f, "b1f"); cs = _req(cs, "colsum")
    b2 = _req(b2, "b2")
    d = x.shape[-1]
    rows = x.numel() // d
    hidden = b1f.numel()
    if stats.dim() != 3 or stats.shape[0] != rows or stats.shape[2] != 2 or wp.numel() != int(_lib.load().cfm_ffn_pack_elems(d, hidden)) or b2.numel() != d:
        raise _lib.ConformerHipError(f"ffn_fused: x(...,{d}), stats{tuple(stats.shape)}, Wp({wp.numel()}), hidden {hidden} do not match")
    y = torch.empty(x.shape, device=x.device, dtype=torch.float32)
    st_out, g2, bt2, eps2, mode = None, None, None, 0.0, 0
    if closing_ln is not None:
        g2 = _req(closing_ln[0], "ln.weight"); bt2 = _req(closing_ln[1], "ln.bias"); eps2 = float(closing_ln[2]); mode = 2
        if emit_stats:
            st_out = torch.empty(rows, 1, 2, device=x.device, dtype=torch.float32)
    elif emit_stats:
        mode = 1
        st_out = torch.empty(rows, d // 32, 2, device=x.device, dtype=torch.float32)
    _lib.check(_lib.load().cfm_ffn_fused_f32(x.data_ptr(), d, stats.data_ptr(), stats.shape[1], float(eps), wp.data_ptr(),
                                             b1f.data_ptr(), cs.data_ptr(), b2.data_ptr(), float(alpha), y.data_ptr(), d, mode,
                                             None if st_out is None else st_out.data_ptr(),
                                             None if g2 is None else g2.data_ptr(), None if bt2 is None else bt2.data_ptr(),
                                             eps2, rows, d, hidden, _stream()), "cfm_ffn_fused_f32")
    return (y, st_out) if emit_stats else y


_ROWCHAIN = __import__("os").environ.get("CONFORMER_AMD_ROWCHAIN", "0") == "1"


def set_rowchain(on: bool) -> bool:
    global _ROWCHAIN
    prev, _ROWCHAIN = _ROWCHAIN, bool(on)
    return prev


def rowchain_ok(d: int, hidden: int, rows: int) -> bool:
    return bool(_ROWCHAIN and ffn_fused_ok(d, hidden, rows))


def rowgemm_pack(w: torch.Tensor, glu: bool = False) -> torch.Tensor:
    w = _req(w.reshape(w.shape[0], -1), "W")
    n, d = w.shape
    wp = torch.empty(n * d, device=w.device, dtype=torch.float32)
    _lib.check(_lib.load().cfm_rowgemm_pack_f32(w.data_ptr(), wp.data_ptr(), n, d, 1 if glu else 0, _stream()), "cfm_rowgemm_pack_f32")
    return wp


def _rowchain(pre, core, post, mode, x, d, *, wpre=None, bpre=None, res=None, y1=None, stats=None, ln_eps=0.0, ffn=None, b2=None,
              alpha=0.0, y=None, stats_out=None, ln2=None, wpost=None, bpost=None, cspost=None, post_eps=0.0, z=None):
    rows = x.numel() // d
    ptr = lambda t: None if t is None else t.data_ptr()
    wp, b1f, cs1 = ffn if ffn is not None else (None, None, None)
    hidden = 0 if b1f is None else b1f.numel()
    g2, bt2, eps2 = ln2 if ln2 is not None else (None, None, 0.0)
    st = _lib.load().cfm_rowchain_f32(pre, core, post, mode, x.data_ptr(), d, ptr(wpre), ptr(bpre), ptr(res), d, ptr(y1), d,
                                      ptr(stats), 0 if stats is None else stats.shape[1], float(ln_eps), ptr(wp), ptr(b1f), ptr(cs1),
                                      ptr(b2), float(alpha), hidden, ptr(y), d, ptr(stats_out), ptr(g2), ptr(bt2), float(eps2),
                                      ptr(wpost), ptr(bpost), ptr(cspost), float(post_eps), ptr(z), 0 if z is None else z.shape[-1],
                                      rows, d, _stream())
    _lib.check(st, "cfm_rowchain_f32")


def rowchain_ffn_qkv(x, stats, ffn, b2, alpha: float, ffn_eps: float, wqkv_p, bqkv_f, csqkv, att_eps: float):
    x = _req(x, "x"); stats = _req(stats, "ln_stats")
    d = x.shape[-1]
    y = torch.empty(x.shape, device=x.device, dtype=torch.float32)
    qkv = torch.empty(*x.shape[:-1], 3 * d, device=x.device, dtype=torch.float32)
    _rowchain(0, 1, 1, 0, x, d, stats=stats, ln_eps=ffn_eps, ffn=ffn, b2=_req(b2, "b2"), alpha=alpha, y=y, wpost=wqkv_p,
              bpost=bqkv_f, cspost=csqkv, post_eps=att_eps, z=qkv)
    return y, qkv


def rowchain_out_glu(ctx, wout_p, bout, res, wglu_p, bglu_f, csglu, conv_eps: float):
    ctx = _req(ctx, "ctx"); res = _req(res, "residual")
    d = ctx.shape[-1]
    y2 = torch.empty(ctx.shape, device=ctx.device, dtype=torch.float32)
    g = torch.empty(ctx.shape, device=ctx.device, dtype=torch.float32)
    _rowchain(1, 0, 2, 0, ctx, d, wpre=wout_p, bpre=_req(bout, "bias"), res=res, y1=y2, ln_eps=conv_eps, wpost=wglu_p, bpost=bglu_f,
              cspost=csglu, z=g)
    return y2, g


def rowchain_pw2_ffn_ln(c, wpw2_p, bpw2, res, ffn, b2, alpha: float, ffn_eps: float, closing_ln, want_stats: bool = False):
    c = _req(c, "c"); res = _req(res, "residual")
    d = c.shape[-1]
    out = torch.empty(c.shape, device=c.device, dtype=torch.float32)
    st = torch.empty(c.numel() // d, 1, 2, device=c.device, dtype=torch.float32) if want_stats else None
    _rowchain(1, 1, 0, 2, c, d, wpre=wpw2_p, bpre=_req(bpw2, "bias"), res=res, ln_eps=ffn_eps, ffn=ffn, b2=_req(b2, "b2"), alpha=alpha,
              y=out, stats_out=st, ln2=(_req(closing_ln[0], "ln.weight"), _req(closing_ln[1], "ln.bias"), float(closing_ln[2])))
    return out, st


def layernorm(x: torch.Tensor, weight: torch.Tensor, bias: torch.Tensor, eps: float = 1e-5,
              out: Optional[torch.Tensor] = None, for_gemm: bool = False, emit_stats: bool = False):
    x = _req(x, "x"); weight = _req(weight, "weight"); bias = _req(bias, "bias")
    d = x.shape[-1]
    rows = x.numel() // d
    if emit_stats:
        y = torch.empty(x.shape, device=x.device, dtype=torch.float32)
        stats = torch.empty(rows, 1, 2, device=x.device, dtype=torch.float32)
        _lib.check(_lib.load().cfm_layernorm_fwd_stats_f32(x.data_ptr(), weight.data_ptr(), bias.data_ptr(), y.data_ptr(),
                                                           stats.data_ptr(), rows, d, eps, _stream()), "cfm_layernorm_fwd_stats_f32")
        return y, stats
    p16 = out16_ok(d) if for_gemm and out is None else 0
    if p16:
        y = torch.empty(x.shape, device=x.device, dtype=_DT16[p16])
        _lib.check(_lib.load().cfm_layernorm_fwd_out16_f32(p16, x.data_ptr(), weight.data_ptr(), bias.data_ptr(), y.data_ptr(),
                                                           None, None, rows, d, eps, _stream()), "cfm_layernorm_fwd_out16_f32")
        return y
    y = _f32_like(x) if out is None else _req(out, "out")
    if y.shape != x.shape:
        raise _lib.ConformerHipError(f"layernorm: out{tuple(y.shape)} does not match x{tuple(x.shape)}")
    st = _lib.load().cfm_layernorm_fwd_f32(x.data_ptr(), weight.data_ptr(), bias.data_ptr(), y.data_ptr(),
                                           None, None, rows, d, eps, _stream())
    _lib.check(st, "cfm_layernorm_fwd_f32")
    return y


def _gemm_common(a: torch.Tensor, w: torch.Tensor, b: torch.Tensor):
    a = _req(a, "A", a.dtype if isinstance(a, torch.Tensor) and a.dtype in _DT16.values() else torch.float32)
    w = _req(w, "W"); b = _req(b, "bias")
    k = a.shape[-1]
    m = a.numel() // k
    w2 = w.reshape(w.shape[0], -1)
    if w2.shape[1] != k:
        raise _lib.ConformerHipError(f"GEMM shape mismatch: A(...,{k}) vs W{tuple(w.shape)}")
    return a, w2, b, m, w2.shape[0], k


def _splitk(m: int, n: int, k: int) -> int:
    tiles = ((m + 63) // 64) * ((n + 63) // 64)
    if tiles > 192 or k < 1024 or n % 4 or m < 1:
        return 0
    return max(2, min(8, k // 512, -(-768 // tiles)))


def _splitk_gemm(epi: int, a, w2, b, c, m, n, k, res=None, alpha: float = 1.0):
    sp = _splitk(m, n, k)
    if not sp or a.dtype != torch.float32 or c.dtype != torch.float32 or _fp32_planes or mfma16_prec():
        return None
    ws = torch.empty(sp * m * n, device=a.device, dtype=torch.float32)
    _lib.check(_lib.load().cfm_gemm_splitk_f32(epi, a.data_ptr(), w2.data_ptr(), b.data_ptr(), _p(res), alpha, c.data_ptr(),
                                               ws.data_ptr(), sp, m, n, k, k, n, n, _stream()), "cfm_gemm_splitk_f32")
    return c


def linear(a, w, b, act: str = "none", for_gemm: bool = False, emit_stats: bool = False):
    a, w2, b, m, n, k = _gemm_common(a, w, b)
    if emit_stats:
        if act != "none" or not ln_fold_ok(n) or a.dtype != torch.float32:
            raise _lib.ConformerHipError("linear(emit_stats=True) needs the native fp32 path, act='none' and ln_fold_ok(N)")
        c = torch.empty(*a.shape[:-1], n, device=a.device, dtype=torch.float32)
        stats = torch.empty(m, n // 32, 2, device=a.device, dtype=torch.float32)
        _lib.check(_lib.load().cfm_gemm_bias_stats_f32(a.data_ptr(), w2.data_ptr(), b.data_ptr(), c.data_ptr(), stats.data_ptr(),
                                                       m, n, k, k, n, _stream()), "cfm_gemm_bias_stats_f32")
        return c, stats
    prec = mfma16_prec()
    p16 = out16_ok(n) if for_gemm else 0
    c = torch.empty(*a.shape[:-1], n, device=a.device, dtype=_DT16[p16] if p16 else torch.float32)
    if prec:
        return _mfma16_gemm(prec, {"none": 0, "swish": 1, "relu": 2}[act], a, w2, b, c, m, n, k)
    if _split_gemm({"none": 0, "swish": 1, "relu": 2}[act], a, w2, b, c, m, n, k) is not None:
        return c
    if act != "relu" and _splitk_gemm({"none": 0, "swish": 1}[act], a, w2, b, c, m, n, k) is not None:
        return c
    fn = {"none": "cfm_gemm_bias_f32", "swish": "cfm_gemm_bias_swish_f32", "relu": "cfm_gemm_bias_relu_f32"}[act]
    st = getattr(_lib.load(), fn)(a.data_ptr(), w2.data_ptr(), b.data_ptr(), c.data_ptr(), m, n, k, k, n, _stream())
    _lib.check(st, fn)
    return c


def linear_glu(a, w, b) -> torch.Tensor:
    a, w2, b, m, n2, k = _gemm_common(a, w, b)
    n = n2 // 2
    c = torch.empty(*a.shape[:-1], n, device=a.device, dtype=torch.float32)
    prec = mfma16_prec()
    if prec:
        return _mfma16_gemm(prec, 3, a, w2, b, c, m, n, k)
    if _split_gemm(3, a, w2, b, c, m, n, k) is not None:
        return c
    st = _lib.load().cfm_gemm_bias_glu_f32(a.data_ptr(), w2.data_ptr(), b.data_ptr(), c.data_ptr(), m, n, k, k, n,
                                           _stream())
    _lib.check(st, "cfm_gemm_bias_glu_f32")
    return c


def linear_residual(a, w, b, res: torch.Tensor, alpha: float = 1.0, emit_stats: bool = False):
    a, w2, b, m, n, k = _gemm_common(a, w, b)
    res = _req(res, "residual")
    if emit_stats:
        if not ln_fold_ok(n) or a.dtype != torch.float32:
            raise _lib.ConformerHipError("linear_residual(emit_stats=True) needs the native fp32 path and ln_fold_ok(N)")
        c = torch.empty(*a.shape[:-1], n, device=a.device, dtype=torch.float32)
        stats = torch.empty(m, n // 32, 2, device=a.device, dtype=torch.float32)
        _lib.check(_lib.load().cfm_gemm_bias_residual_stats_f32(a.data_ptr(), w2.data_ptr(), b.data_ptr(), res.data_ptr(), alpha,
                                                                c.data_ptr(), stats.data_ptr(), m, n, k, k, n, n, _stream()),
                   "cfm_gemm_bias_residual_stats_f32")
        return c, stats
    c = torch.empty(*a.shape[:-1], n, device=a.device, dtype=torch.float32)
    prec = mfma16_prec()
    if prec:
        return _mfma16_gemm(prec, 4, a, w2, b, c, m, n, k, res, alpha)
    if _split_gemm(4, a, w2, b, c, m, n, k, res, alpha) is not None:
        return c
    if _splitk_gemm(4, a, w2, b, c, m, n, k, res, alpha) is not None:
        return c
    st = _lib.load().cfm_gemm_bias_residual_f32(a.data_ptr(), w2.data_ptr(), b.data_ptr(), res.data_ptr(), alpha,
                                                c.data_ptr(), m, n, k, k, n, n, _stream())
    _lib.check(st, "cfm_gemm_bias_residual_f32")
    return c


def relpos_table(div_term: torch.Tensor, t: int) -> torch.Tensor:
    dt = _req(div_term, "div_term").reshape(-1)
    d = 2 * dt.numel()
    pe = torch.empty(2 * t - 1, d, device=dt.device, dtype=torch.float32)
    st = _lib.load().cfm_relpos_table_f32(dt.data_ptr(), pe.data_ptr(), t, d, _stream())
    _lib.check(st, "cfm_relpos_table_f32")
    return pe


def _req_pos(pos: torch.Tensor, T: int, d: int) -> None:
    if not (isinstance(pos, torch.Tensor) and pos.is_cuda and pos.dtype == torch.float32 and pos.dim() == 2
            and pos.stride(1) == 1 and pos.shape == (2 * T - 1, d)):
        raise _lib.ConformerHipError(f"pos: expected a ({2 * T - 1},{d}) fp32 HIP tensor with unit column stride")


def _key_split(B: int, n_heads: int, q_rows: int, T: int, keys_hint: Optional[int]) -> int:
    tiles = ((T if keys_hint is None else min(int(keys_hint), T)) + 31) // 32
    blocks = B * n_heads * ((q_rows + 127) // 128)
    return max(1, min(16, tiles // 8, -(-1024 // blocks)))


def _key_split16(B: int, n_heads: int, q_rows: int, T: int, keys_hint: Optional[int]) -> int:
    tiles = ((T if keys_hint is None else min(int(keys_hint), T)) + 31) // 32
    blocks = B * n_heads * ((q_rows + 127) // 128)
    return max(1, min(16, tiles // 8, 512 // blocks))


def relpos_attention(qkv: torch.Tensor, pos: torch.Tensor, u: torch.Tensor, v: torch.Tensor,
                     lengths: Optional[torch.Tensor], n_heads: int, for_gemm: bool = False) -> torch.Tensor:
    u = _req(u, "content_bias"); v = _req(v, "position_bias")
    prec = mfma16_prec()
    q16 = bool(prec) and isinstance(qkv, torch.Tensor) and qkv.dtype == _DT16[prec]
    if q16:
        if not (qkv.is_cuda and qkv.is_contiguous() and qkv.shape[-1] % 24 == 0):
            raise _lib.ConformerHipError("16-bit qkv: expected a contiguous HIP tensor with d % 8 == 0")
    else:
        qkv = _req(qkv, "qkv")
    B, T, d3 = qkv.shape
    d = d3 // 3
    dh = d // n_heads
    _req_pos(pos, T, d)
    ldp = pos.stride(0)
    if lengths is not None:
        lengths = _req(lengths, "lengths", torch.int64)
    base = qkv.data_ptr()
    c16 = bool(prec and for_gemm and d % 8 == 0)
    if q16 or c16:
        esz = 2 if q16 else 4
        ctx = torch.empty(B, T, d, device=qkv.device, dtype=_DT16[prec] if c16 else torch.float32)
        st = _lib.load().cfm_relpos_attention_io16_mfma16_f32(prec, base, base + esz * d, base + 2 * esz * d, int(q16), d3,
                                                              pos.data_ptr(), ldp, u.data_ptr(), v.data_ptr(), _p(lengths),
                                                              ctx.data_ptr(), int(c16), d, B, T, n_heads, dh, _stream())
        _lib.check(st, "cfm_relpos_attention_io16_mfma16_f32")
        return ctx
    ctx = torch.empty(B, T, d, device=qkv.device, dtype=torch.float32)
    if prec:
        st = _lib.load().cfm_relpos_attention_mfma16_f32(prec, base, base + 4 * d, base + 8 * d, d3, pos.data_ptr(), ldp,
                                                         u.data_ptr(), v.data_ptr(), _p(lengths), ctx.data_ptr(), d, None,
                                                         B, T, n_heads, dh, 0.0, 0, _stream())
        _lib.check(st, "cfm_relpos_attention_mfma16_f32")
        return ctx
    st = _lib.load().cfm_relpos_attention_fwd_f32(base, base + 4 * d, base + 8 * d, d3, pos.data_ptr(), ldp,
                                                  u.data_ptr(), v.data_ptr(), _p(lengths), ctx.data_ptr(), d, None,
                                                  B, T, n_heads, dh, _stream())
    _lib.check(st, "cfm_relpos_attention_fwd_f32")
    return ctx


def relpos_attention_rows(qkv: torch.Tensor, pos: torch.Tensor, u: torch.Tensor, v: torch.Tensor, lengths: torch.Tensor,
                          n_heads: int, q_begin: int, q_count: int, ctx: torch.Tensor, keys_hint: Optional[int] = None
                          ) -> torch.Tensor:
    qkv = _req(qkv, "qkv"); u = _req(u, "content_bias"); v = _req(v, "position_bias"); ctx = _req(ctx, "ctx")
    B, T, d3 = qkv.shape
    d = d3 // 3
    _req_pos(pos, T, d)
    if ctx.shape != (B, T, d) or not qkv.is_contiguous() or not ctx.is_contiguous():
        raise _lib.ConformerHipError("relpos_attention_rows: qkv (B,T,3d) and ctx (B,T,d) must be contiguous cache buffers")
    lengths = _req(lengths, "lengths", torch.int64)
    prec = mfma16_prec()
    if prec != PREC_F32:
        base = qkv.data_ptr()
        st = _lib.load().cfm_relpos_attention_rows_mfma16_f32(prec, base, base + 4 * d, base + 8 * d, d3, pos.data_ptr(), pos.stride(0),
                                                              u.data_ptr(), v.data_ptr(), lengths.data_ptr(), ctx.data_ptr(), d, B, T,
                                                              n_heads, d // n_heads, int(q_begin), int(q_count), _stream())
        _lib.check(st, "cfm_relpos_attention_rows_mfma16_f32")
        return ctx
    nsplit = _key_split(B, n_heads, q_count, T, keys_hint)
    ws = torch.empty(nsplit * B * q_count * (d + n_heads), device=qkv.device, dtype=torch.float32) if nsplit > 1 else None
    base = qkv.data_ptr()
    st = _lib.load().cfm_relpos_attention_rows_f32(base, base + 4 * d, base + 8 * d, d3, pos.data_ptr(), pos.stride(0),
                                                   u.data_ptr(), v.data_ptr(), lengths.data_ptr(), ctx.data_ptr(), d, B, T,
                                                   n_heads, d // n_heads, int(q_begin), int(q_count), nsplit, _p(ws), _stream())
    _lib.check(st, "cfm_relpos_attention_rows_f32")
    return ctx


def relpos_attention_slots(qkv: torch.Tensor, pos: torch.Tensor, u: torch.Tensor, v: torch.Tensor, lengths: torch.Tensor,
                           n_heads: int, q_begin: torch.Tensor, q_count: torch.Tensor, q_max: int,
                           ctx: Optional[torch.Tensor] = None, keys_hint: Optional[int] = None) -> torch.Tensor:
    u = _req(u, "content_bias"); v = _req(v, "position_bias")
    prec = mfma16_prec()
    q16 = isinstance(qkv, torch.Tensor) and qkv.dtype in (torch.bfloat16, torch.float16)
    if q16:
        if not prec or qkv.dtype != _DT16[prec]:
            raise _lib.ConformerHipError(f"relpos_attention_slots: a {qkv.dtype} cache needs torch.autocast of that type")
        if not (qkv.is_cuda and qkv.dim() == 3 and qkv.shape[-1] % 24 == 0):
            raise _lib.ConformerHipError("relpos_attention_slots: 16-bit qkv: expected a (S,T,3d) HIP tensor with d % 8 == 0")
    else:
        qkv = _req(qkv, "qkv")
    B, T, d3 = qkv.shape
    d = d3 // 3
    q_max = int(q_max)
    _req_pos(pos, T, d)
    if not qkv.is_contiguous():
        raise _lib.ConformerHipError("relpos_attention_slots: qkv (S,T,3d) must be a contiguous cache buffer")
    if ctx is None:
        ctx = torch.empty(B, q_max, d, device=qkv.device, dtype=torch.float32)
    ctx = _req(ctx, "ctx")
    if ctx.shape != (B, q_max, d) or not ctx.is_contiguous():
        raise _lib.ConformerHipError(f"relpos_attention_slots: ctx must be a contiguous ({B},{q_max},{d}) tensor")
    lengths = _req(lengths, "lengths", torch.int64)
    q_begin = _req(q_begin, "q_begin", torch.int64)
    q_count = _req(q_count, "q_count", torch.int64)
    for name, t in (("lengths", lengths), ("q_begin", q_begin), ("q_count", q_count)):
        if t.shape != (B,) or not t.is_contiguous():
            raise _lib.ConformerHipError(f"relpos_attention_slots: {name} must be a contiguous ({B},) int64 tensor")
    nsplit = (_key_split16 if prec else _key_split)(B, n_heads, q_max, T, keys_hint)
    ws = torch.empty(nsplit * B * q_max * (d + n_heads), device=qkv.device, dtype=torch.float32) if nsplit > 1 else None
    base = qkv.data_ptr()
    if prec != PREC_F32:
        esz = 2 if q16 else 4
        st = _lib.load().cfm_relpos_attention_slots_mfma16_f32(prec, base, base + esz * d, base + 2 * esz * d, int(q16), d3,
                                                               pos.data_ptr(), pos.stride(0), u.data_ptr(), v.data_ptr(),
                                                               q_begin.data_ptr(), q_count.data_ptr(), lengths.data_ptr(),
                                                               ctx.data_ptr(), d, B, T, n_heads, d // n_heads, q_max, nsplit,
                                                               _p(ws), _stream())
        _lib.check(st, "cfm_relpos_attention_slots_mfma16_f32")
        return ctx
    st = _lib.load().cfm_relpos_attention_slots_f32(base, base + 4 * d, base + 8 * d, d3, pos.data_ptr(), pos.stride(0),
                                                    u.data_ptr(), v.data_ptr(), q_begin.data_ptr(), q_count.data_ptr(),
                                                    lengths.data_ptr(), ctx.data_ptr(), d, B, T, n_heads, d // n_heads, q_max,
                                                    nsplit, _p(ws), _stream())
    _lib.check(st, "cfm_relpos_attention_slots_f32")
    return ctx


def dwconv_bn_swish(g, w, b, bn_w, bn_b, bn_mean, bn_var, eps: float = 1e-5, for_gemm: bool = False) -> torch.Tensor:
    g = _req(g, "g"); w = _req(w, "dw weight"); b = _req(b, "dw bias")
    B, T, C = g.shape
    K = w.shape[-1]
    p16 = out16_ok(C) if for_gemm and K in (3, 7, 15, 31) else 0
    if p16:
        y = torch.empty(g.shape, device=g.device, dtype=_DT16[p16])
        st = _lib.load().cfm_dwconv_bn_swish_fwd_out16_f32(p16, g.data_ptr(), w.data_ptr(), b.data_ptr(), _req(bn_w, "bn_w").data_ptr(),
                                                           _req(bn_b, "bn_b").data_ptr(), _req(bn_mean, "bn_mean").data_ptr(),
                                                           _req(bn_var, "bn_var").data_ptr(), eps, y.data_ptr(), B, T, C, K,
                                                           _stream())
        _lib.check(st, "cfm_dwconv_bn_swish_fwd_out16_f32")
        return y
    y = _f32_like(g)
    st = _lib.load().cfm_dwconv_bn_swish_fwd_f32(g.data_ptr(), w.data_ptr(), b.data_ptr(), _req(bn_w, "bn_w").data_ptr(),
                                                 _req(bn_b, "bn_b").data_ptr(), _req(bn_mean, "bn_mean").data_ptr(),
                                                 _req(bn_var, "bn_var").data_ptr(), eps, y.data_ptr(), B, T, C, K,
                                                 _stream())
    _lib.check(st, "cfm_dwconv_bn_swish_fwd_f32")
    return y


_CONVMOD_FUSED = __import__("os").environ.get("CONFORMER_AMD_CONVMOD_FUSED", "1") != "0"
_CONVMOD_MIN_ROW_EFF = 0.875


def set_convmod_fused(on: bool) -> bool:
    global _CONVMOD_FUSED
    prev, _CONVMOD_FUSED = _CONVMOD_FUSED, bool(on)
    return prev


def convmod_chunks(T: int, K: int) -> int:
    return 1 if T <= 256 else 1 + (T - 256 + (256 - K)) // (257 - K)

# ... 729 lines not shown
```

### include/conformer_hip.h

```cpp
#ifndef CONFORMER_HIP_H
#define CONFORMER_HIP_H

#include <stddef.h>
#include <stdint.h>

#ifdef __cplusplus
extern "C" {
#endif

typedef void* cfm_stream_t;

enum cfm_status {
    CFM_OK = 0,
    CFM_ERR_BAD_SHAPE = -1,
    CFM_ERR_UNSUPPORTED = -2,
    CFM_ERR_NULL = -3,
    CFM_ERR_LAUNCH = -4,
    CFM_ERR_DEVICE = -5,
    CFM_ERR_ALIGN = -6
};

int cfm_version(void);
int cfm_abi_version(void);
#define CFM_ABI_VERSION 4
const char* cfm_strerror(int status);
int cfm_device_check(void);

int cfm_layernorm_fwd_f32(const float* x, const float* gamma, const float* beta, float* y,
                          float* mean_or_null, float* rstd_or_null,
                          int64_t rows, int d, float eps, cfm_stream_t stream);

int cfm_gemm_bias_f32(const float* A, const float* W, const float* bias, float* C,
                      int64_t M, int N, int K, int64_t lda, int64_t ldc, cfm_stream_t stream);
int cfm_gemm_bias_swish_f32(const float* A, const float* W, const float* bias, float* C,
                            int64_t M, int N, int K, int64_t lda, int64_t ldc, cfm_stream_t stream);
int cfm_gemm_bias_relu_f32(const float* A, const float* W, const float* bias, float* C,
                           int64_t M, int N, int K, int64_t lda, int64_t ldc, cfm_stream_t stream);
int cfm_gemm_bias_glu_f32(const float* A, const float* W, const float* bias, float* C,
                          int64_t M, int n_out, int K, int64_t lda, int64_t ldc, cfm_stream_t stream);
int cfm_gemm_bias_residual_f32(const float* A, const float* W, const float* bias, const float* R,
                               float alpha, float* C, int64_t M, int N, int K,
                               int64_t lda, int64_t ldr, int64_t ldc, cfm_stream_t stream);

int cfm_gemm_splitk_f32(int epi, const float* A, const float* W, const float* bias, const float* R_or_null,
                        float alpha, float* C, float* workspace, int splits, int64_t M, int N, int K,
                        int64_t lda, int64_t ldr, int64_t ldc, cfm_stream_t stream);

int cfm_gemm_bias_stats_f32(const float* A, const float* W, const float* bias, float* C, float* stats_out,
                            int64_t M, int N, int K, int64_t lda, int64_t ldc, cfm_stream_t stream);
int cfm_gemm_bias_residual_stats_f32(const float* A, const float* W, const float* bias, const float* R,
                                     float alpha, float* C, float* stats_out, int64_t M, int N, int K,
                                     int64_t lda, int64_t ldr, int64_t ldc, cfm_stream_t stream);
int cfm_gemm_lnfold_f32(int epi, const float* A, const float* ln_stats, int ln_parts, float ln_eps,
                        const float* Wf, const float* bias_f, const float* colsum, float* C,
                        int64_t M, int N, int K, int64_t lda, int64_t ldc, cfm_stream_t stream);
int cfm_layernorm_fwd_stats_f32(const float* x, const float* gamma, const float* beta, float* y,
                                float* stats_out, int64_t rows, int d, float eps, cfm_stream_t stream);

int64_t cfm_ffn_pack_elems(int d, int hidden);
int cfm_ffn_pack_f32(const float* W1f, const float* W2, float* Wp, int d, int hidden, cfm_stream_t stream);
int cfm_ffn_fused_f32(const float* X, int64_t ldx, const float* ln_stats, int ln_parts, float ln_eps, const float* Wp,
                      const float* b1f, const float* colsum1, const float* b2, float alpha, float* Y, int64_t ldy,
                      int mode, float* stats_out, const float* gamma2, const float* beta2, float eps2, int64_t M,
                      int d, int hidden, cfm_stream_t stream);

int cfm_rowgemm_pack_f32(const float* W, float* Wp, int N, int d, int glu, cfm_stream_t stream);
int cfm_rowchain_f32(int pre, int core, int post, int mode, const float* X, int64_t ldx, const float* Wpre_packed,
                     const float* bpre, const float* R, int64_t ldr, float* Y1, int64_t ldy1, const float* ln_stats,
                     int ln_parts, float ln_eps, const float* Wffn_packed, const float* b1f, const float* colsum1,
                     const float* b2, float alpha, int hidden, float* Y, int64_t ldy, float* stats_out,
                     const float* gamma2, const float* beta2, float eps2, const float* Wpost_packed, const float* bpost,
                     const float* cspost, float post_eps, float* Z, int64_t ldz, int64_t M, int d, cfm_stream_t stream);
int64_t cfm_ffn_tile_stride_f4(int d);
int cfm_ffn_rotate(void);

int cfm_relpos_table_f32(const float* div_term, float* pe, int T, int d, cfm_stream_t stream);

int cfm_relpos_attention_fwd_f32(const float* q, const float* k, const float* v, int64_t ld,
                                 const float* pos, int64_t ldp, const float* u, const float* vbias,
                                 const int64_t* lengths_or_null, float* ctx, int64_t ldo,
                                 float* lse_or_null, int B, int T, int H, int dh, cfm_stream_t stream);

int cfm_dwconv_bn_swish_fwd_f32(const float* g, const float* w, const float* bias,
                                const float* bn_weight, const float* bn_bias,
                                const float* bn_mean, const float* bn_var, float bn_eps,
                                float* y, int B, int T, int C, int K, cfm_stream_t stream);

int cfm_convmod_glu_dwconv_f32(const float* x, int64_t ldx, const float* ln_stats, int ln_parts, float ln_eps,
                               const float* Wf, const float* bias_f, const float* colsum, const float* dw_w,
                               const float* dw_b, const float* bn_w, const float* bn_b, const float* bn_mean,
                               const float* bn_var, float bn_eps, float* y, int64_t ldy, int B, int T, int C, int K,
                               cfm_stream_t stream);

int cfm_subsample_conv1_relu_f32(const float* x, const float* w1, const float* b1, float* h1,
                                 int B, int F, int T, int C, cfm_stream_t stream);
int cfm_pack_conv2_weight_f32(const float* w2, float* w2p, int C, cfm_stream_t stream);
int cfm_subsample_conv2_relu_f32(const float* h1, const float* w2p, const float* b2, float* h2,
                                 int B, int F1, int T1, int C, cfm_stream_t stream);
int cfm_pack_linear_weight_f32(const float* wl, float* wlp, int d_out, int C, int F2, cfm_stream_t stream);
int64_t cfm_conv2_wino_plane_elems(int B, int F1, int T1, int C);
int cfm_pack_conv2_wino_weight_f32(const float* w2, float* wwp, int C, cfm_stream_t stream);
int cfm_subsample_conv2_wino_relu_f32(const float* h1, const float* wwp, const float* b2, float* planes, float* h2,
                                      int B, int F1, int T1, int C, cfm_stream_t stream);

#define CFM_PREC_F32 0
#define CFM_PREC_BF16 1
#define CFM_PREC_FP16 2
int cfm_gemm_mfma16_f32(int prec, int epi, const void* A, int a_is_16bit, const void* W, int w_is_16bit,
                        const float* bias, const float* R_or_null, float alpha, void* C, int c_is_16bit,
                        void* Z_or_null, int z_is_16bit, int64_t M, int N, int K, int64_t lda, int64_t ldr,
                        int64_t ldc, float drop_p, uint64_t drop_seed, cfm_stream_t stream);
#define CFM_CAST_BATCH 48
typedef struct cfm_cast_item {
    const float* src;
    void* dst;
    int64_t rows, cols;
    int transpose;
} cfm_cast_item;
int cfm_cast16_multi_f32(int prec, const cfm_cast_item* items, int count, cfm_stream_t stream);
int cfm_layernorm_fwd_out16_f32(int prec, const float* x, const float* gamma, const float* beta, void* y16,
                                float* mean_or_null, float* rstd_or_null, int64_t rows, int d, float eps,
                                cfm_stream_t stream);
int cfm_cast16_f32(int prec, const float* src, void* dst, int64_t n, cfm_stream_t stream);
int cfm_relpos_attention_mfma16_f32(int prec, const float* q, const float* k, const float* v, int64_t ld,
                                    const float* pos, int64_t ldp, const float* u, const float* vbias,
                                    const int64_t* lengths_or_null, float* ctx, int64_t ldo, float* lse_or_null, int B,
                                    int T, int H, int dh, float drop_p, uint64_t drop_seed, cfm_stream_t stream);
int cfm_relpos_attention_rows_mfma16_f32(int prec, const float* q, const float* k, const float* v, int64_t ld,
                                         const float* pos, int64_t ldp, const float* u, const float* vbias,
                                         const int64_t* lengths, float* ctx, int64_t ldo, int B, int T, int H, int dh,
                                         int q_begin, int q_count, cfm_stream_t stream);
int cfm_relpos_attention_io16_mfma16_f32(int prec, const void* q, const void* k, const void* v, int qkv_is_16bit, int64_t ld,
                                         const float* pos, int64_t ldp, const float* u, const float* vbias,
                                         const int64_t* lengths_or_null, void* ctx, int ctx_is_16bit, int64_t ldo, int B, int T,
                                         int H, int dh, cfm_stream_t stream);
int cfm_subsample_conv2_relu_mfma16_f32(int prec, const void* h1, int h1_is_16bit, const void* w2p, int w_is_16bit,
                                        const float* b2, void* h2, int h2_is_16bit, int B, int F1, int T1, int C,
                                        cfm_stream_t stream);
int cfm_subsample_conv1_relu_out16_f32(int prec, const float* x, const float* w1, const float* b1, void* h1, int B, int F,
                                       int T, int C, cfm_stream_t stream);
int cfm_gemm_bwd_batched_mfma16_f32(int prec, const float* A, int a_col, int64_t lda, const void* B, int b_col,
                                    int b_is_16bit, int64_t ldb, const void* Z_or_null, int z_is_16bit, int64_t ldz, float alpha, void* C,
                                    int64_t ldc, int c_is_16bit, int I, int J, int64_t Kc, int allow_split, int accumulate,
                                    int nbatch, int nb1, int64_t sa0, int64_t sa1, int64_t sb0, int64_t sb1,
                                    int64_t sc0, int64_t sc1, float drop_p, uint64_t drop_seed,
                                    int operands_zero_padded4, cfm_stream_t stream);
int cfm_linear_bwd_weight_mfma16_f32(int prec, const void* dy, int dy_is_16bit, int64_t ldy, const void* x,
                                     int x_is_16bit, int64_t ldx, float* dw, int64_t ldw, float* db_or_null, int N,
                                     int K, int64_t M, float alpha, cfm_stream_t stream);
int64_t cfm_subsample_conv2_rowtab_elems(int B, int F1, int T1);
int cfm_subsample_conv2_bwd_weight_h16_mfma16_f32(int prec, const void* dz2, int dz2_is_16bit, const void* h1_16,
                                                  int* rowtab_scratch, float* dw2p, float* db2_or_null, int B, int F1, int T1,
                                                  int C, cfm_stream_t stream);
int cfm_dwconv_bn_swish_fwd_out16_f32(int prec, const float* g, const float* w, const float* bias, const float* bn_weight,
                                      const float* bn_bias, const float* bn_mean, const float* bn_var, float bn_eps,
                                      void* y16, int B, int T, int C, int K, cfm_stream_t stream);
int cfm_glu_bwd_out16_f32(int prec, const float* z, const float* dy, void* dz16, int64_t rows, int n, cfm_stream_t stream);
int cfm_relu_bwd_out16_f32(int prec, const float* y, const float* dy, void* dz16, int64_t n, cfm_stream_t stream);
int cfm_subsample_conv2_bwd_input_fwdkernel_mfma16_f32(int prec, const void* dz2, int dz2_is_16bit, const void* w2c16,
                                                       const float* zero_bias, float* dh1, int B, int F1, int T1,
                                                       int C, cfm_stream_t stream);
int cfm_subsample_conv2_bwd_input_fwdkernel_out16_mfma16_f32(int prec, const void* dz2, int dz2_is_16bit, const void* w2c16,
                                                             const float* zero_bias, void* dh1_16, int B, int F1, int T1, int C,
                                                             cfm_stream_t stream);
int cfm_subsample_conv1_bwd_d16_f32(int prec, const float* x, const float* w1, const float* b1, const void* dh1_16, float* dw1,
                                    float* db1, int B, int F, int T, int C, cfm_stream_t stream);
int cfm_subsample_conv2_bwd_weight_mfma16_f32(int prec, const float* dz2, const float* h1, float* dw2p, int B, int F1,
                                              int T1, int C, cfm_stream_t stream);
int cfm_subsample_conv2_bwd_input_mfma16_f32(int prec, const float* dz2, const float* w2c, float* dh1, int B, int F1,
                                             int T1, int C, cfm_stream_t stream);

int cfm_reflect_pad_f32(const float* x, float* xp, int B, int64_t L, int pad, int64_t ld_out, cfm_stream_t stream);
int cfm_power_mel_log_f32(const float* spec, int64_t ld_spec, const float* fb, float* out, int B, int T,
                          int n_bins, int n_mels, float floor_value, cfm_stream_t stream);
int cfm_power_mel_log_mfma_f32(const float* spec, int64_t ld_spec, const float* fbT, float* out, int B, int T,
                               int rows_per_utt, int n_bins, int n_mels, float floor_value, cfm_stream_t stream);
int cfm_dft_frames_f32(const float* wave, const float* basis, float* spec, int64_t rows, int n_cols, int n_fft,
                       int hop, cfm_stream_t stream);
int cfm_specaugment_apply_f32(float* spec, int B, int F, int T, const int* bands, int nbands, float value,
                              cfm_stream_t stream);


int cfm_gemm_bias_swish_save_f32(const float* A, const float* W, const float* bias, float* C, float* Z,
                                 int64_t M, int N, int K, int64_t lda, int64_t ldc, cfm_stream_t stream);

int cfm_gemm_bwd_f32(const float* A, int a_col, int64_t lda, const float* B, int b_col, int64_t ldb,
                     const float* Z_or_null, int64_t ldz, float alpha, float* C, int64_t ldc,
                     int I, int J, int64_t Kc, int allow_split, cfm_stream_t stream);
int cfm_gemm_bwd_batched_f32(const float* A, int a_col, int64_t lda, const float* B, int b_col, int64_t ldb,
                             const float* Z_or_null, int64_t ldz, float alpha, float* C, int64_t ldc,
                             int I, int J, int64_t Kc, int allow_split, int accumulate, int nbatch, int nb1,
                             int64_t sa0, int64_t sa1, int64_t sb0, int64_t sb1, int64_t sc0, int64_t sc1,
                             float drop_p, uint64_t drop_seed, cfm_stream_t stream);

int cfm_gemm_train_f32(int epi, const float* A, const float* W, const float* bias, const float* R_or_null,
                       float alpha, float* C, float* Z_or_null, int64_t M, int N, int K, int64_t lda,
                       int64_t ldr, int64_t ldc, float drop_p, uint64_t drop_seed, cfm_stream_t stream);
int cfm_relpos_attention_train_f32(const float* q, const float* k, const float* v, int64_t ld,
                                   const float* pos, int64_t ldp, const float* u, const float* vbias,
                                   const int64_t* lengths_or_null, float* ctx, int64_t ldo, float* lse,
                                   int B, int T, int H, int dh, float drop_p, uint64_t drop_seed,
                                   cfm_stream_t stream);
int cfm_dropout_f32(const float* x, float* y, int64_t n, float p, uint64_t seed, cfm_stream_t stream);
int cfm_dropout_out16_f32(int prec, const float* x, void* y16, int64_t n, float p, uint64_t seed, cfm_stream_t stream);

int cfm_layernorm_bwd_dx_f32(const float* x, const float* gamma, const float* dy, const float* mean,
                             const float* rstd, const float* dres_or_null, float* dx, int64_t rows, int d,
                             cfm_stream_t stream);
int cfm_layernorm_bwd_params_f32(const float* x, const float* dy, const float* mean, const float* rstd,
                                 float* dgamma, float* dbeta, int64_t rows, int d, cfm_stream_t stream);
size_t cfm_layernorm_bwd_workspace_bytes(int64_t rows, int d);
int cfm_layernorm_bwd_f32(const float* x, const float* gamma, const float* dy, const float* mean,
                          const float* rstd, const float* dres_or_null, float* dx, float* dgamma, float* dbeta,
                          int64_t rows, int d, void* workspace, size_t workspace_bytes, cfm_stream_t stream);

int cfm_colsum_f32(const float* X, int64_t ld, int64_t rows, int cols, float alpha, float* out,
                   cfm_stream_t stream);

int cfm_glu_fwd_f32(const float* z, float* y, int64_t rows, int n, cfm_stream_t stream);
int cfm_glu_bwd_f32(const float* z, const float* dy, float* dz, int64_t rows, int n, cfm_stream_t stream);

int cfm_dwconv_bn_swish_bwd_f32(const float* g, const float* dy, const float* w, const float* bias,
                                const float* bn_weight, const float* bn_bias, const float* bn_mean,
                                const float* bn_var, float bn_eps, int train_stats, float* dc_ws, float* dg,
                                float* dw, float* dbias, float* dgamma, float* dbeta, int B, int T, int C,
                                int K, cfm_stream_t stream);

size_t cfm_dwconv_bn_stats_workspace_bytes(int B, int T, int C);
int cfm_dwconv_bn_stats_f32(const float* g, const float* w, const float* bias, float* batch_mean,
                            float* batch_var, float* running_mean_or_null, float* running_var_or_null,
                            float momentum, int B, int T, int C, int K, void* workspace, size_t workspace_bytes,
                            cfm_stream_t stream);

int cfm_relpos_attention_bwd_f32(const float* q, const float* k, const float* v, int64_t ld, const float* pos,
                                 int64_t ldp, const float* u, const float* vbias, const int64_t* lengths_or_null,
                                 const float* ctx, const float* dctx, int64_t ldo, const float* lse, float* dq,
                                 float* dk, float* dv, int64_t ldg, float* dpos, int64_t lddp, float* du,
                                 float* dvbias, int B, int T, int H, int dh, float drop_p, uint64_t drop_seed,
                                 int prec, cfm_stream_t stream);

int cfm_relpos_attention_bwd_mfma16_f32(int prec, const float* q, const float* k, const float* v, int64_t ld,
                                        const float* pos, int64_t ldp, const float* u, const float* vbias,
                                        const int64_t* lengths_or_null, const float* ctx, const float* dctx, int64_t ldo,
                                        const float* lse, float* dq, float* dk, float* dv, int64_t ldg, float* dpos,
                                        int64_t lddp, float* du, float* dvbias, int B, int T, int H, int dh,
                                        float drop_p, uint64_t drop_seed, cfm_stream_t stream);

int cfm_debug_attention_bwd_trace_f32(void* trace_or_null);
int cfm_debug_attention_bwd_trace_mfma16(void* trace_or_null);
int cfm_debug_dw16_trace(void* trace_or_null);
int cfm_debug_lstm_trace(void* trace_or_null);
int cfm_debug_gemm_mfma16_force_tile(int tile);
int cfm_debug_gemm_mfma16_trace(void* trace_or_null);
int cfm_debug_gemm_last_tile(int family, int* out);

int cfm_debug_gemm_cfg_f32(int cfg, const float* A, const float* W, const float* bias, const float* R,
                           float alpha, float* C, int64_t M, int N, int K, void* trace_or_null,
                           cfm_stream_t stream);
int cfm_debug_ffn_trace(void* trace_or_null, int per_slice);
int cfm_debug_ffn_variant(int v);
int cfm_debug_convmod_variant(int v);
int cfm_debug_ffn_layout(int pad_f4, int rotate);
int cfm_debug_set_conv2_bk(int bk);

int cfm_relu_bwd_f32(const float* y, const float* dy, float* dz, int64_t n, cfm_stream_t stream);
int cfm_subsample_conv2_bwd_weight_f32(const float* dz2, const float* h1, float* dw2p, int B, int F1, int T1,
                                       int C, cfm_stream_t stream);
int cfm_pack_conv2_weight_t_f32(const float* w2, float* w2c, int C, cfm_stream_t stream);
int cfm_subsample_conv2_bwd_input_f32(const float* dz2, const float* w2c, float* dh1, int B, int F1, int T1,
                                      int C, cfm_stream_t stream);
int cfm_subsample_conv1_bwd_f32(const float* x, const float* w1, const float* b1, const float* dh1, float* dw1,
                                float* db1, int B, int F, int T, int C, cfm_stream_t stream);

typedef struct cfm_adam_tensor {
    float* param;
    const float* grad;
    float* exp_avg;
    float* exp_avg_sq;
    int64_t numel;
} cfm_adam_tensor;
int cfm_adam_step_f32(const cfm_adam_tensor* tensors, int n_tensors, float lr, float beta1, float beta2, float eps,
                      float bias_c1, float sqrt_bias_c2, cfm_stream_t stream);
int cfm_greedy_ctc_decode_f32(const float* logits, const int64_t* lengths_or_null, int64_t* frame_ids,
                              int64_t* tokens, int64_t* counts, int B, int T, int V, int pad_id, int unk_id,
                              cfm_stream_t stream);

size_t cfm_ctc_beam_workspace_bytes(int B, int T, int W, int K);
int cfm_ctc_beam_decode_f32(const float* logits, const int64_t* lengths_or_null, int B, int T, int V, int blank_id,
                            int beam_width, int max_candidates, float token_min_logp, float beam_prune_logp, int n_best,
                            void* workspace, size_t workspace_bytes, int64_t* tokens, int64_t* counts, float* scores,
                            int64_t* num_hyps, cfm_stream_t stream);

size_t cfm_ngram_lm_pack_bytes(int order, const int64_t* ngram_counts, int n_words, int64_t word_cp_total, int V,
                               int64_t tok_cp_total);
int cfm_ngram_lm_pack(int order, const int64_t* ngram_counts, const int32_t* ngram_words, const float* ngram_logp,
                      const float* ngram_backoff, int n_words, const int64_t* word_cp_offsets, const int32_t* word_cp, int bos_id,
                      int eos_id, int unk_id, int V, const int64_t* tok_cp_offsets, const int32_t* tok_cp, const int32_t* tok_kind,
                      void* out, size_t out_bytes);
int cfm_ngram_lm_score_f64(const void* lm_tables, const int32_t* words, const int64_t* offsets, int n_sentences, int boundary,
                           double* out, cfm_stream_t stream);
size_t cfm_ctc_beam_lm_workspace_bytes(int B, int T, int W, int K);
int cfm_ctc_beam_lm_decode_f32(const float* logits, const int64_t* lengths_or_null, int B, int T, int V, int blank_id,
                               int beam_width, int max_candidates, float token_min_logp, float beam_prune_logp, int n_best,
                               const void* lm_tables, double alpha, double beta, double unk_score_offset, int score_boundary,
                               void* workspace, size_t workspace_bytes, int64_t* tokens, int64_t* counts, float* scores,
                               float* am_scores, int64_t* num_hyps, cfm_stream_t stream);

size_t cfm_hotword_pack_bytes(int n_unigrams, int64_t uni_cp_total, int n_phrases, int64_t phrase_word_total, int V,
                              int64_t tok_cp_total);
int cfm_hotword_pack(int n_unigrams, const int64_t* uni_cp_offsets, const int32_t* uni_cp, int n_phrases,
                     const int64_t* phrase_offsets, const int32_t* phrase_words, int V, const int64_t* tok_cp_offsets,
                     const int32_t* tok_cp, const int32_t* tok_kind, void* out, size_t out_bytes);
int cfm_hotword_count(const void* hw_tables, const int32_t* tokens, const int64_t* offsets, int n_seqs, double weight,
                      int32_t* counts, double* bonus, int32_t* final_counts);
size_t cfm_ctc_beam_hw_workspace_bytes(int B, int T, int W, int K);
int cfm_ctc_beam_hw_decode_f32(const float* logits, const int64_t* lengths_or_null, int B, int T, int V, int blank_id,
                               int beam_width, int max_candidates, float token_min_logp, float beam_prune_logp, int n_best,
                               const void* lm_tables_or_null, double alpha, double beta, double unk_score_offset,
                               int score_boundary, const void* hw_tables, double hotword_weight, void* workspace,
                               size_t workspace_bytes, int64_t* tokens, int64_t* counts, float* scores, float* am_scores,
                               int64_t* num_hyps, cfm_stream_t stream);

size_t cfm_ctc_beam_stream_state_bytes(int B, int T_max, int W, int K, int lm, int hw);
int cfm_ctc_beam_stream_init(int B, int T_max, int beam_width, int max_candidates, const void* lm_tables_or_null,
                             int score_boundary, const void* hw_tables_or_null, void* state, size_t state_bytes,
                             cfm_stream_t stream);
int cfm_ctc_beam_stream_step_f32(const float* logits, const int64_t* lengths_or_null, int B, int Tc, int V, int blank_id,
                                 int beam_width, int max_candidates, float token_min_logp, float beam_prune_logp, int n_best,
                                 const void* lm_tables_or_null, double alpha, double beta, double unk_score_offset,
                                 int score_boundary, const void* hw_tables_or_null, double hotword_weight, void* state,
                                 size_t state_bytes, int T_max, int t_used, int64_t* tokens, int64_t* counts, float* scores,
                                 float* am_scores_or_null, int64_t* num_hyps, cfm_stream_t stream);
int cfm_ctc_beam_stream_finish_f32(int B, int beam_width, int max_candidates, int n_best, const void* lm_tables_or_null,
                                   double alpha, double beta, double unk_score_offset, int score_boundary,
                                   const void* hw_tables_or_null, double hotword_weight, void* state, size_t state_bytes,
                                   int T_max, int64_t* tokens, int64_t* counts, float* scores, float* am_scores_or_null,
                                   int64_t* num_hyps, cfm_stream_t stream);
int cfm_ctc_beam_stream_reset_slots(int B, int T_max, int beam_width, int max_candidates, const void* lm_tables_or_null,
                                    int score_boundary, const void* hw_tables_or_null, const int64_t* slots, int n_slots,
                                    void* state, size_t state_bytes, cfm_stream_t stream);

int cfm_lstm_fwd_f32(const float* gates_x, const float* w_hh, const int64_t* lengths_or_null, float* y, float* c_state,
                     float* save_gates_or_null, float* save_c_or_null, int B, int T, int H, cfm_stream_t stream);
int cfm_lstm_bwd_f32(const float* dy, const float* gates, const float* cells, const float* whh_t,
                     const int64_t* lengths_or_null, float* dgates, float* dc_state, int B, int T, int H,
                     cfm_stream_t stream);
int cfm_lstm_fwd_frag_f32(const float* gates_x, const float* w_hh_frag, const int64_t* lengths_or_null, float* y,
                          float* c_state, float* h_frag_scratch, float* save_gates_or_null, float* save_c_or_null, int B,
                          int T, int H, cfm_stream_t stream);
int cfm_lstm_bwd_frag_f32(const float* dy, const float* gates, const float* cells, const float* whh_t_frag,
                          const int64_t* lengths_or_null, float* dgates, float* dc_state, float* dg_frag_scratch, int B,
                          int T, int H, cfm_stream_t stream);
int cfm_lstm_fwd_mfma16_f32(int prec, const float* gates_x, const void* w_hh16, const int64_t* lengths_or_null, float* y,
                            float* c_state, void* h16_scratch, float* save_gates_or_null, float* save_c_or_null, int B,
                            int T, int H, cfm_stream_t stream);
int cfm_lstm_fwd_carry_f32(const float* gates_x, const float* w_hh, const int64_t* lengths_or_null, float* y, float* h_state,
                           float* c_state, float* save_gates_or_null, float* save_c_or_null, int B, int T, int H,
                           cfm_stream_t stream);
int cfm_lstm_fwd_frag_carry_f32(const float* gates_x, const float* w_hh_frag, const int64_t* lengths_or_null, float* y,
                                float* h_state, float* c_state, float* h_frag_scratch, float* save_gates_or_null,
                                float* save_c_or_null, int B, int T, int H, cfm_stream_t stream);
int cfm_lstm_fwd_mfma16_carry_f32(int prec, const float* gates_x, const void* w_hh16, const int64_t* lengths_or_null, float* y,
                                  float* h_state, float* c_state, void* h16_scratch, float* save_gates_or_null,
                                  float* save_c_or_null, int B, int T, int H, cfm_stream_t stream);
int cfm_lstm_bwd_mfma16_f32(int prec, const float* dy, const float* gates, const float* cells, const void* whh_t16,
                            const int64_t* lengths_or_null, float* dgates, float* dc_state, void* dg16_scratch, int B,
                            int T, int H, cfm_stream_t stream);
int cfm_swish_bn_eval_f32(const float* h, const float* bn_mean, const float* bn_var, const float* bn_weight,
                          const float* bn_bias, float eps, float* out, int64_t rows, int C, cfm_stream_t stream);
int cfm_swish_bn_stats_f32(const float* h, float* batch_mean, float* batch_var, float* running_mean_or_null,
                           float* running_var_or_null, float momentum, int64_t rows, int C, cfm_stream_t stream);
int cfm_swish_bn_bwd_f32(const float* h, const float* dz, const float* bn_mean, const float* bn_var,
                         const float* bn_weight, float eps, int train_stats, float* dh, float* dgamma, float* dbeta,
                         int64_t rows, int C, cfm_stream_t stream);

// ... 56 lines not shown
```

Before: 1.719 million audio-frames/sec.

## Fuse block seam: pw2, FFN2, closing LN, next block FFN1 and QKV into one kernel

Adds a seam_chain kernel that chains the conv pointwise-2 projection, the second feed-forward, the block's closing LayerNorm, the next block's first feed-forward and its LN-folded QKV projection, keeping each 32-row tile in shared memory and registers across block boundaries. The feed-forward core is factored into an includable stage header so it can be instantiated twice per kernel. The aim is to remove several kernel launches and the global-memory round trips of intermediate activations between blocks. In exchange the kernel holds more state per block and is larger, so register pressure and longer single-kernel latency could offset the savings.

```diff
diff --git a/conformer_amd/_lib.py b/conformer_amd/_lib.py
--- a/conformer_amd/_lib.py
+++ b/conformer_amd/_lib.py
@@ -23,6 +23,8 @@
     "cfm_rowgemm_pack_f32": (c_int, [_P, _P, _I, _I, _I, _P]),
     "cfm_rowchain_f32": (c_int, [_I, _I, _I, _I, _P, _L, _P, _P, _P, _L, _P, _L, _P, _I, _F, _P, _P, _P, _P, _F, _I, _P, _L, _P, _P, _P, _F,
                                  _P, _P, _P, _F, _P, _L, _L, _I, _P]),
+    "cfm_seam_chain_f32": (c_int, [_P, _L, _P, _P, _P, _L, _F, _P, _P, _P, _P, _F, _P, _P, _F, _F, _P, _P, _P, _P, _F, _I, _P, _L, _P, _P, _P, _F,
+                                   _P, _L, _L, _I, _P]),
     "cfm_ffn_tile_stride_f4": (ctypes.c_int64, [_I]),
     "cfm_ffn_rotate": (c_int, []),
     "cfm_ffn_fused_f32": (c_int, [_P, _L, _P, _I, _F, _P, _P, _P, _P, _F, _P, _L, _I, _P, _P, _P, _F, _L, _I, _I, _P]),
diff --git a/conformer_amd/csrc/rowchain_core_stage.h b/conformer_amd/csrc/rowchain_core_stage.h
--- /dev/null
+++ b/conformer_amd/csrc/rowchain_core_stage.h
@@ -0,0 +1,213 @@
+        const int NS = a.hidden >> 7;
+        const f32x4* wp = reinterpret_cast<const f32x4*>(CORE_WP) + lane;
+        const int64_t TILE = a.tile_stride;
+        const int rot = a.rotate ? (int)((blockIdx.x >> 3) % (unsigned)NS) : 0;
+        f32x4 ring[RING];
+        {
+            const f32x4* sb = wp + (4 * rot + wave) * TILE;
+#pragma unroll
+            for (int i = 0; i < RING; ++i) ring[i] = sb[i * 64];
+        }
+#pragma unroll
+        for (int t = 0; t < ND; ++t)
+#pragma unroll
+            for (int r = 0; r < 16; ++r) y[t][r] = 0.f;
+        for (int s = 0; s < NS; ++s) {
+            const int sr = s + rot < NS ? s + rot : s + rot - NS;
+            const int g = 4 * sr + wave;
+            const f32x4* sb = wp + g * TILE;
+            const f32x4* nb = wp + (4 * (sr + 1 < NS ? sr + 1 : 0) + wave) * TILE;
+            f32x4 csv[4], b1v[4];
+#pragma unroll
+            for (int q = 0; q < 4; ++q) {
+                csv[q] = *reinterpret_cast<const f32x4*>(CORE_CS1 + g * 32 + 8 * q + 4 * hf);
+                b1v[q] = *reinterpret_cast<const f32x4*>(CORE_B1F + g * 32 + 8 * q + 4 * hf);
+            }
+            f32x16 ha;
+#pragma unroll
+            for (int r = 0; r < 16; ++r) ha[r] = 0.f;
+            f32x4 xv = *reinterpret_cast<const f32x4*>(xrow);
+#pragma unroll
+            for (int c = 0; c < NL; ++c) {
+                const f32x4 xn = *reinterpret_cast<const f32x4*>(xrow + 8 * (c + 1));
+                const f32x4 wv = ring[c % RING];
+                ring[c % RING] = sb[(c + RING) * 64];
+                ha = __builtin_amdgcn_mfma_f32_32x32x2f32(wv[0], xv[0], ha, 0, 0, 0);
+                ha = __builtin_amdgcn_mfma_f32_32x32x2f32(wv[1], xv[1], ha, 0, 0, 0);
+                ha = __builtin_amdgcn_mfma_f32_32x32x2f32(wv[2], xv[2], ha, 0, 0, 0);
+                ha = __builtin_amdgcn_mfma_f32_32x32x2f32(wv[3], xv[3], ha, 0, 0, 0);
+                xv = xn;
+                __builtin_amdgcn_sched_barrier(0);
+            }
+            float sw[16];
+#pragma unroll
+            for (int r = 0; r < 16; ++r) {
+                const float v = rstd * (ha[r] - mean * csv[r >> 2][r & 3]) + b1v[r >> 2][r & 3];
+                sw[r] = swishf_acc(v);
+            }
+#pragma unroll
+            for (int j = 0; j < NL; j += 2) {
+                const int q = j / ND, t = j % ND;
+                const f32x4 w0 = ring[j % RING], w1 = ring[(j + 1) % RING];
+                ring[j % RING] = j + RING < NL ? sb[(NL + j + RING) * 64] : nb[(j + RING - NL) * 64];
+                ring[(j + 1) % RING] = j + 1 + RING < NL ? sb[(NL + j + 1 + RING) * 64] : nb[(j + 1 + RING - NL) * 64];
+#pragma unroll
+                for (int e = 0; e < 4; ++e) {
+                    y[t] = __builtin_amdgcn_mfma_f32_32x32x2f32(w0[e], sw[4 * q + e], y[t], 0, 0, 0);
+                    y[t + 1] = __builtin_amdgcn_mfma_f32_32x32x2f32(w1[e], sw[4 * q + e], y[t + 1], 0, 0, 0);
+                }
+                __builtin_amdgcn_sched_barrier(0);
+            }
+        }
+
+        float* Ex = Ys;
+        const bool cok = 4 * li < QW;
+        const int cl = cok ? 4 * li : 0;
+        f32x4 v[4][4];
+#pragma unroll
+        for (int c = 0; c < 4; ++c) {
+#pragma unroll
+            for (int k = 0; k < TPW; ++k)
+#pragma unroll
+                for (int q = 0; q < 4; ++q)
+                    *reinterpret_cast<f32x4*>(Ex + wave * ERS + li * EW + 32 * k + 8 * q + 4 * hf) =
+                        f32x4{y[c * TPW + k][4 * q], y[c * TPW + k][4 * q + 1], y[c * TPW + k][4 * q + 2], y[c * TPW + k][4 * q + 3]};
+            const f32x4 b2v = *reinterpret_cast<const f32x4*>(CORE_B2 + QW * c + cl);
+            __syncthreads();
+#pragma unroll
+            for (int it = 0; it < 4; ++it) {
+                const int r = 8 * wave + 2 * it + hf;
+                const float* e = Ex + r * EW + cl;
+                f32x4 acc = *reinterpret_cast<const f32x4*>(e);
+                acc += *reinterpret_cast<const f32x4*>(e + ERS);
+                acc += *reinterpret_cast<const f32x4*>(e + 2 * ERS);
+                acc += *reinterpret_cast<const f32x4*>(e + 3 * ERS);
+                const f32x4 xr = *reinterpret_cast<const f32x4*>(Xs + r * XS + QW * c + cl);
+                v[c][it] = cok ? CORE_ALPHA * (acc + b2v) + xr : f32x4{0.f, 0.f, 0.f, 0.f};
+            }
+            __syncthreads();
+        }
+        auto half_sum = [](float (&t)[4]) {
+#pragma unroll
+            for (int o = 16; o > 0; o >>= 1)
+#pragma unroll
+                for (int it = 0; it < 4; ++it) t[it] += __shfl_xor(t[it], o, 64);
+        };
+        if constexpr (CORE_FIN == CH_LN) {
+            f32x4 gam[4], bet[4];
+#pragma unroll
+            for (int c = 0; c < 4; ++c) {
+                gam[c] = *reinterpret_cast<const f32x4*>(a.gamma2 + QW * c + cl);
+                bet[c] = *reinterpret_cast<const f32x4*>(a.beta2 + QW * c + cl);
+            }
+            float s[4], q[4];
+#pragma unroll
+            for (int it = 0; it < 4; ++it) {
+                s[it] = 0.f;
+#pragma unroll
+                for (int c = 0; c < 4; ++c) s[it] += (v[c][it][0] + v[c][it][1]) + (v[c][it][2] + v[c][it][3]);
+            }
+            half_sum(s);
+#pragma unroll
+            for (int it = 0; it < 4; ++it) {
+                const float mu = s[it] * (1.0f / (float)D);
+                q[it] = 0.f;
+#pragma unroll
+                for (int c = 0; c < 4; ++c) {
+                    if (cok) {
+                        v[c][it] = v[c][it] - mu;
+                        q[it] += (v[c][it][0] * v[c][it][0] + v[c][it][1] * v[c][it][1]) + (v[c][it][2] * v[c][it][2] + v[c][it][3] * v[c][it][3]);
+                    }
+                }
+            }
+            half_sum(q);
+#pragma unroll
+            for (int it = 0; it < 4; ++it) {
+                const float rs = 1.0f / sqrtf(q[it] * (1.0f / (float)D) + a.eps2);
+                s[it] = 0.f;
+#pragma unroll
+                for (int c = 0; c < 4; ++c) {
+                    if (cok) {
+                        v[c][it] = v[c][it] * rs * gam[c] + bet[c];
+                        s[it] += (v[c][it][0] + v[c][it][1]) + (v[c][it][2] + v[c][it][3]);
+                    }
+                }
+            }
+            if (a.stats_out) {
+                half_sum(s);
+#pragma unroll
+                for (int it = 0; it < 4; ++it) {
+                    const float mo = s[it] * (1.0f / (float)D);
+                    q[it] = 0.f;
+#pragma unroll
+                    for (int c = 0; c < 4; ++c) {
+                        if (cok) {
+                            const f32x4 tt = v[c][it] - mo;
+                            q[it] += (tt[0] * tt[0] + tt[1] * tt[1]) + (tt[2] * tt[2] + tt[3] * tt[3]);
+                        }
+                    }
+                }
+                half_sum(q);
+#pragma unroll
+                for (int it = 0; it < 4; ++it) {
+                    const int64_t row = m0 + 8 * wave + 2 * it + hf;
+                    if (li == 0 && row < a.M) *reinterpret_cast<float2*>(a.stats_out + 2 * row) = float2{s[it], q[it]};
+                }
+            }
+        }
+        if constexpr (CORE_KEEP) {
+            float s[4], q[4];
+#pragma unroll
+            for (int it = 0; it < 4; ++it) {
+                s[it] = 0.f;
+#pragma unroll
+                for (int c = 0; c < 4; ++c) {
+                    s[it] += (v[c][it][0] + v[c][it][1]) + (v[c][it][2] + v[c][it][3]);
+                    if (cok) *reinterpret_cast<f32x4*>(Xs + (8 * wave + 2 * it + hf) * XS + QW * c + cl) = v[c][it];
+                }
+            }
+            half_sum(s);
+#pragma unroll
+            for (int it = 0; it < 4; ++it) {
+                const float mu = s[it] * (1.0f / (float)D);
+                q[it] = 0.f;
+#pragma unroll
+                for (int c = 0; c < 4; ++c) {
+                    if (cok) {
+                        const f32x4 dv = v[c][it] - mu;
+                        q[it] += (dv[0] * dv[0] + dv[1] * dv[1]) + (dv[2] * dv[2] + dv[3] * dv[3]);
+                    }
+                }
+                s[it] = mu;
+            }
+            half_sum(q);
+#pragma unroll
+            for (int it = 0; it < 4; ++it)
+                if (li == 0) {
+                    St[2 * (8 * wave + 2 * it + hf)] = s[it];
+                    St[2 * (8 * wave + 2 * it + hf) + 1] = 1.0f / sqrtf(q[it] * (1.0f / (float)D) + CORE_KEEP_EPS);
+                }
+        }
+#pragma unroll
+        for (int it = 0; it < 4; ++it) {
+            const int64_t row = m0 + 8 * wave + 2 * it + hf;
+            const bool row_ok = row < a.M;
+#pragma unroll
+            for (int c = 0; c < 4; ++c) {
+                if (CORE_STORE && row_ok && cok) *reinterpret_cast<f32x4*>(a.Y + row * a.ldy + QW * c + cl) = v[c][it];
+                if constexpr (CORE_FIN == CH_STATS) {
+                    float s = (v[c][it][0] + v[c][it][1]) + (v[c][it][2] + v[c][it][3]);
+                    s += __shfl_xor(s, 1, 64); s += __shfl_xor(s, 2, 64); s += __shfl_xor(s, 4, 64);
+                    const float m = s * (1.0f / 32.0f);
+                    const f32x4 dv = v[c][it] - m;
+                    float q = (dv[0] * dv[0] + dv[1] * dv[1]) + (dv[2] * dv[2] + dv[3] * dv[3]);
+                    q += __shfl_xor(q, 1, 64); q += __shfl_xor(q, 2, 64); q += __shfl_xor(q, 4, 64);
+                    if (row_ok && cok && (li & 7) == 0)
+                        *reinterpret_cast<float2*>(a.stats_out + (row * (int64_t)ND + ((QW * c + cl) >> 5)) * 2) = float2{s, q};
+                }
+            }
+        }
+        if constexpr (CORE_KEEP) {
+            __syncthreads();
+            mean = St[2 * li]; rstd = St[2 * li + 1];
+        }
diff --git a/conformer_amd/csrc/rowchain_f32.hip b/conformer_amd/csrc/rowchain_f32.hip
--- a/conformer_amd/csrc/rowchain_f32.hip
+++ b/conformer_amd/csrc/rowchain_f32.hip
@@ -13,17 +13,19 @@
     float* Y; int64_t ldy; float* stats_out; const float* gamma2; const float* beta2; float eps2;
     const float* Wpost; const float* bpost; const float* cspost; float post_eps; float* Z; int64_t ldz;
     int64_t M;
+    const float* Wp_b; const float* b1f_b; const float* cs1_b; const float* b2_b; float alpha_b; float eps_b;
 };
 
 enum { CH_PLAIN = 0, CH_STATS = 1, CH_LN = 2 };
 enum { POST_NONE = 0, POST_BIAS3 = 1, POST_GLU = 2 };
 
-template <int ND, int PRE, int CORE, int POST, int MODE>
+template <int ND, int PRE, int CORE, int POST, int MODE, int SEAM = 0>
 __global__ __launch_bounds__(256, 1) void rowchain_f32_kernel(const ChainArgs a) {
     constexpr int D = 32 * ND, XS = D + 4, NL = 4 * ND, RING = 16;
     constexpr int TPW = ND / 4, QW = 32 * TPW, EW = QW + 4, ERS = 32 * EW;
     static_assert(NL % RING == 0 && ND % 4 == 0, "d = 128, 256 or 512");
     static_assert(CORE || (PRE && POST), "a chain without the feed-forward is PRE + POST");
+    static_assert(!SEAM || (PRE && CORE), "the seam is PRE + two feed-forwards (+ POST)");
     __shared__ __attribute__((aligned(16))) float smem[32 * XS + 4 * ERS + 64];
     float* Xs = smem;
     float* Ys = smem + 32 * XS;
@@ -153,220 +155,69 @@
         row_stats(a.ln_eps, a.Y1, a.ldy1);
     }
 
-    if constexpr (CORE) {
-        const int NS = a.hidden >> 7;
-        const f32x4* wp = reinterpret_cast<const f32x4*>(a.Wp) + lane;
-        const int64_t TILE = a.tile_stride;
-        const int rot = a.rotate ? (int)((blockIdx.x >> 3) % (unsigned)NS) : 0;
-        f32x4 ring[RING];
+    if constexpr (CORE && SEAM) {
         {
-            const f32x4* sb = wp + (4 * rot + wave) * TILE;
-#pragma unroll
-            for (int i = 0; i < RING; ++i) ring[i] = sb[i * 64];
-        }
-#pragma unroll
-        for (int t = 0; t < ND; ++t)
-#pragma unroll
-            for (int r = 0; r < 16; ++r) y[t][r] = 0.f;
-        for (int s = 0; s < NS; ++s) {
-            const int sr = s + rot < NS ? s + rot : s + rot - NS;
-            const int g = 4 * sr + wave;
-            const f32x4* sb = wp + g * TILE;
-            const f32x4* nb = wp + (4 * (sr + 1 < NS ? sr + 1 : 0) + wave) * TILE;
-            f32x4 csv[4], b1v[4];
-#pragma unroll
-            for (int q = 0; q < 4; ++q) {
-                csv[q] = *reinterpret_cast<const f32x4*>(a.cs1 + g * 32 + 8 * q + 4 * hf);
-                b1v[q] = *reinterpret_cast<const f32x4*>(a.b1f + g * 32 + 8 * q + 4 * hf);
-            }
-            f32x16 ha;
-#pragma unroll
-            for (int r = 0; r < 16; ++r) ha[r] = 0.f;
-            f32x4 xv = *reinterpret_cast<const f32x4*>(xrow);
-#pragma unroll
-            for (int c = 0; c < NL; ++c) {
-                const f32x4 xn = *reinterpret_cast<const f32x4*>(xrow + 8 * (c + 1));
-                const f32x4 wv = ring[c % RING];
-                ring[c % RING] = sb[(c + RING) * 64];
-                ha = __builtin_amdgcn_mfma_f32_32x32x2f32(wv[0], xv[0], ha, 0, 0, 0);
-                ha = __builtin_amdgcn_mfma_f32_32x32x2f32(wv[1], xv[1], ha, 0, 0, 0);
-                ha = __builtin_amdgcn_mfma_f32_32x32x2f32(wv[2], xv[2], ha, 0, 0, 0);
-                ha = __builtin_amdgcn_mfma_f32_32x32x2f32(wv[3], xv[3], ha, 0, 0, 0);
-                xv = xn;
-                __builtin_amdgcn_sched_barrier(0);
-            }
-            float sw[16];
-#pragma unroll
-            for (int r = 0; r < 16; ++r) {
-                const float v = rstd * (ha[r] - mean * csv[r >> 2][r & 3]) + b1v[r >> 2][r & 3];
-                sw[r] = swishf_acc(v);
-            }
-#pragma unroll
-            for (int j = 0; j < NL; j += 2) {
-                const int q = j / ND, t = j % ND;
-                const f32x4 w0 = ring[j % RING], w1 = ring[(j + 1) % RING];
-                ring[j % RING] = j + RING < NL ? sb[(NL + j + RING) * 64] : nb[(j + RING - NL) * 64];
-                ring[(j + 1) % RING] = j + 1 + RING < NL ? sb[(NL + j + 1 + RING) * 64] : nb[(j + 1 + RING - NL) * 64];
-#pragma unroll
-                for (int e = 0; e < 4; ++e) {
-                    y[t] = __builtin_amdgcn_mfma_f32_32x32x2f32(w0[e], sw[4 * q + e], y[t], 0, 0, 0);
-                    y[t + 1] = __builtin_amdgcn_mfma_f32_32x32x2f32(w1[e], sw[4 * q + e], y[t + 1], 0, 0, 0);
-                }
-                __builtin_amdgcn_sched_barrier(0);
-            }
-        }
-
-        float* Ex = Ys;
-        const bool cok = 4 * li < QW;
-        const int cl = cok ? 4 * li : 0;
-        f32x4 v[4][4];
-#pragma unroll
-        for (int c = 0; c < 4; ++c) {
-#pragma unroll
-            for (int k = 0; k < TPW; ++k)
-#pragma unroll
-                for (int q = 0; q < 4; ++q)
-                    *reinterpret_cast<f32x4*>(Ex + wave * ERS + li * EW + 32 * k + 8 * q + 4 * hf) =
-                        f32x4{y[c * TPW + k][4 * q], y[c * TPW + k][4 * q + 1], y[c * TPW + k][4 * q + 2], y[c * TPW + k][4 * q + 3]};
-            const f32x4 b2v = *reinterpret_cast<const f32x4*>(a.b2 + QW * c + cl);
-            __syncthreads();
-#pragma unroll
-            for (int it = 0; it < 4; ++it) {
-                const int r = 8 * wave + 2 * it + hf;
-                const float* e = Ex + r * EW + cl;
-                f32x4 acc = *reinterpret_cast<const f32x4*>(e);
-                acc += *reinterpret_cast<const f32x4*>(e + ERS);
-                acc += *reinterpret_cast<const f32x4*>(e + 2 * ERS);
-                acc += *reinterpret_cast<const f32x4*>(e + 3 * ERS);
-                const f32x4 xr = *reinterpret_cast<const f32x4*>(Xs + r * XS + QW * c + cl);
-                v[c][it] = cok ? a.alpha * (acc + b2v) + xr : f32x4{0.f, 0.f, 0.f, 0.f};
-            }
-            __syncthreads();
-        }
-        auto half_sum = [](float (&t)[4]) {
-#pragma unroll
-            for (int o = 16; o > 0; o >>= 1)
-#pragma unroll
-                for (int it = 0; it < 4; ++it) t[it] += __shfl_xor(t[it], o, 64);
-        };
-        if constexpr (POST) {
-            float s[4], q[4];
-#pragma unroll
-            for (int it = 0; it < 4; ++it) {
-                s[it] = 0.f;
-#pragma unroll
-                for (int c = 0; c < 4; ++c) {
-                    s[it] += (v[c][it][0] + v[c][it][1]) + (v[c][it][2] + v[c][it][3]);
-                    if (cok) *reinterpret_cast<f32x4*>(Xs + (8 * wave + 2 * it + hf) * XS + QW * c + cl) = v[c][it];
-                }
-            }
-            half_sum(s);
-#pragma unroll
-            for (int it = 0; it < 4; ++it) {
-                const float mu = s[it] * (1.0f / (float)D);
-                q[it] = 0.f;
-#pragma unroll
-                for (int c = 0; c < 4; ++c) {
-                    if (cok) {
-                        const f32x4 dv = v[c][it] - mu;
-                        q[it] += (dv[0] * dv[0] + dv[1] * dv[1]) + (dv[2] * dv[2] + dv[3] * dv[3]);
-                    }
-                }
-                s[it] = mu;
-            }
-            half_sum(q);
-#pragma unroll
-            for (int it = 0; it < 4; ++it)
-                if (li == 0) {
-                    St[2 * (8 * wave + 2 * it + hf)] = s[it];
-                    St[2 * (8 * wave + 2 * it + hf) + 1] = 1.0f / sqrtf(q[it] * (1.0f / (float)D) + a.post_eps);
-                }
-        }
-        if constexpr (MODE == CH_LN) {
-            f32x4 gam[4], bet[4];
-#pragma unroll
-            for (int c = 0; c < 4; ++c) {
-                gam[c] = *reinterpret_cast<const f32x4*>(a.gamma2 + QW * c + cl);
-                bet[c] = *reinterpret_cast<const f32x4*>(a.beta2 + QW * c + cl);
-            }
-            float s[4], q[4];
-#pragma unroll
-            for (int it = 0; it < 4; ++it) {
-                s[it] = 0.f;
-#pragma unroll
-                for (int c = 0; c < 4; ++c) s[it] += (v[c][it][0] + v[c][it][1]) + (v[c][it][2] + v[c][it][3]);
-            }
-            half_sum(s);
-#pragma unroll
-            for (int it = 0; it < 4; ++it) {
-                const float mu = s[it] * (1.0f / (float)D);
-                q[it] = 0.f;
-#pragma unroll
-                for (int c = 0; c < 4; ++c) {
-                    if (cok) {
-                        v[c][it] = v[c][it] - mu;
-                        q[it] += (v[c][it][0] * v[c][it][0] + v[c][it][1] * v[c][it][1]) + (v[c][it][2] * v[c][it][2] + v[c][it][3] * v[c][it][3]);
-                    }
-                }
-            }
-            half_sum(q);
-#pragma unroll
-            for (int it = 0; it < 4; ++it) {
-                const float rs = 1.0f / sqrtf(q[it] * (1.0f / (float)D) + a.eps2);
-                s[it] = 0.f;
-#pragma unroll
-                for (int c = 0; c < 4; ++c) {
-                    if (cok) {
-                        v[c][it] = v[c][it] * rs * gam[c] + bet[c];
-                        s[it] += (v[c][it][0] + v[c][it][1]) + (v[c][it][2] + v[c][it][3]);
-                    }
-                }
-            }
-            if (a.stats_out) {
-                half_sum(s);
-#pragma unroll
-                for (int it = 0; it < 4; ++it) {
-                    const float mo = s[it] * (1.0f / (float)D);
-                    q[it] = 0.f;
-#pragma unroll
-                    for (int c = 0; c < 4; ++c) {
-                        if (cok) {
-                            const f32x4 tt = v[c][it] - mo;
-                            q[it] += (tt[0] * tt[0] + tt[1] * tt[1]) + (tt[2] * tt[2] + tt[3] * tt[3]);
-                        }
-                    }
-                }
-                half_sum(q);
-#pragma unroll
-                for (int it = 0; it < 4; ++it) {
-                    const int64_t row = m0 + 8 * wave + 2 * it + hf;
-                    if (li == 0 && row < a.M) *reinterpret_cast<float2*>(a.stats_out + 2 * row) = float2{s[it], q[it]};
-                }
-            }
-        }
-#pragma unroll
-        for (int it = 0; it < 4; ++it) {
-            const int64_t row = m0 + 8 * wave + 2 * it + hf;
-            const bool row_ok = row < a.M;
-#pragma unroll
-            for (int c = 0; c < 4; ++c) {
-                if (row_ok && cok) *reinterpret_cast<f32x4*>(a.Y + row * a.ldy + QW * c + cl) = v[c][it];
-                if constexpr (MODE == CH_STATS) {
-                    float s = (v[c][it][0] + v[c][it][1]) + (v[c][it][2] + v[c][it][3]);
-                    s += __shfl_xor(s, 1, 64); s += __shfl_xor(s, 2, 64); s += __shfl_xor(s, 4, 64);
-                    const float m = s * (1.0f / 32.0f);
-                    const f32x4 dv = v[c][it] - m;
-                    float q = (dv[0] * dv[0] + dv[1] * dv[1]) + (dv[2] * dv[2] + dv[3] * dv[3]);
-                    q += __shfl_xor(q, 1, 64); q += __shfl_xor(q, 2, 64); q += __shfl_xor(q, 4, 64);
-                    if (row_ok && cok && (li & 7) == 0)
-                        *reinterpret_cast<float2*>(a.stats_out + (row * (int64_t)ND + ((QW * c + cl) >> 5)) * 2) = float2{s, q};
-                }
-            }
-        }
-        if constexpr (POST) {
-            __syncthreads();
-            mean = St[2 * li]; rstd = St[2 * li + 1];
-        }
+#define CORE_WP a.Wp
+#define CORE_B1F a.b1f
+#define CORE_CS1 a.cs1
+#define CORE_B2 a.b2
+#define CORE_ALPHA a.alpha
+#define CORE_FIN CH_LN
+#define CORE_KEEP true
+#define CORE_KEEP_EPS a.eps_b
+#define CORE_STORE false
+#include "rowchain_core_stage.h"
+#undef CORE_WP
+#undef CORE_B1F
+#undef CORE_CS1
+#undef CORE_B2
+#undef CORE_ALPHA
+#undef CORE_FIN
+#undef CORE_KEEP
+#undef CORE_KEEP_EPS
+#undef CORE_STORE
+        }
+        {
+#define CORE_WP a.Wp_b
+#define CORE_B1F a.b1f_b
+#define CORE_CS1 a.cs1_b
+#define CORE_B2 a.b2_b
+#define CORE_ALPHA a.alpha_b
+#define CORE_FIN MODE
+#define CORE_KEEP (POST != POST_NONE)
+#define CORE_KEEP_EPS a.post_eps
+#define CORE_STORE true
+#include "rowchain_core_stage.h"
+#undef CORE_WP
+#undef CORE_B1F
+#undef CORE_CS1
+#undef CORE_B2
+#undef CORE_ALPHA
+#undef CORE_FIN
+#undef CORE_KEEP
+#undef CORE_KEEP_EPS
+#undef CORE_STORE
+        }
+    } else if constexpr (CORE) {
+#define CORE_WP a.Wp
+#define CORE_B1F a.b1f
+#define CORE_CS1 a.cs1
+#define CORE_B2 a.b2
+#define CORE_ALPHA a.alpha
+#define CORE_FIN MODE
+#define CORE_KEEP (POST != POST_NONE)
+#define CORE_KEEP_EPS a.post_eps
+#define CORE_STORE true
+#include "rowchain_core_stage.h"
+#undef CORE_WP
+#undef CORE_B1F
+#undef CORE_CS1
+#undef CORE_B2
+#undef CORE_ALPHA
+#undef CORE_FIN
+#undef CORE_KEEP
+#undef CORE_KEEP_EPS
+#undef CORE_STORE
     }
 
     if constexpr (POST != POST_NONE) {
@@ -484,7 +335,7 @@
     if (M == 0) return CFM_OK;
     ChainArgs a{X, ldx, Wpre_packed, bpre, R, ldr, Y1, ldy1, ln_stats, ln_parts, ln_eps, Wffn_packed, b1f, colsum1, b2, alpha, hidden,
                 cfm_ffn_tile_stride_f4(d), cfm_ffn_rotate(), Y, ldy, stats_out, gamma2, beta2, eps2, Wpost_packed, bpost, cspost,
-                post_eps, Z, ldz, M};
+                post_eps, Z, ldz, M, nullptr, nullptr, nullptr, nullptr, 0.f, 0.f};
     const dim3 grid((unsigned)((M + 31) / 32)), block(256);
     hipStream_t s = static_cast<hipStream_t>(stream);
 #define CH_LAUNCH(ND, PRE, CORE, POST, MODE) hipLaunchKernelGGL((rowchain_f32_kernel<ND, PRE, CORE, POST, MODE>), grid, block, 0, s, a)
@@ -498,3 +349,31 @@
 #undef CH_LAUNCH
     return cfm_launch_status();
 }
+
+extern "C" int cfm_seam_chain_f32(const float* C, int64_t ldc, const float* Wpw2_packed, const float* bpw2, const float* R, int64_t ldr,
+                                  float ffn2_eps, const float* Wffn2_packed, const float* b1f2, const float* colsum2, const float* b2_2,
+                                  float alpha2, const float* gamma, const float* beta, float ln_eps, float ffn1_eps,
+                                  const float* Wffn1_packed, const float* b1f1, const float* colsum1, const float* b2_1, float alpha1,
+                                  int hidden, float* Y, int64_t ldy, const float* Wqkv_packed, const float* bqkv, const float* csqkv,
+                                  float att_eps, float* Z, int64_t ldz, int64_t M, int d, cfm_stream_t stream) {
+    CFM_REQUIRE(C && M >= 0 && ldc >= d && ldc % 4 == 0 && CFM_ALIGNED16(C), CFM_ERR_BAD_SHAPE);
+    CFM_REQUIRE(d == 128 || d == 256 || d == 512, CFM_ERR_UNSUPPORTED);
+    CFM_REQUIRE(hidden > 0 && hidden % 128 == 0, CFM_ERR_UNSUPPORTED);
+    CFM_REQUIRE(Wpw2_packed && bpw2 && R && Wffn2_packed && b1f2 && colsum2 && b2_2 && gamma && beta && Wffn1_packed && b1f1 && colsum1 &&
+                b2_1 && Y && Wqkv_packed && bqkv && csqkv && Z, CFM_ERR_NULL);
+    CFM_REQUIRE(ldr >= d && ldr % 4 == 0 && ldy >= d && ldy % 4 == 0 && ldz >= 3 * d && ldz % 4 == 0, CFM_ERR_ALIGN);
+    CFM_REQUIRE(CFM_ALIGNED16(Wpw2_packed) && CFM_ALIGNED16(bpw2) && CFM_ALIGNED16(R) && CFM_ALIGNED16(Wffn2_packed) && CFM_ALIGNED16(b1f2) &&
+                CFM_ALIGNED16(colsum2) && CFM_ALIGNED16(b2_2) && CFM_ALIGNED16(gamma) && CFM_ALIGNED16(beta) && CFM_ALIGNED16(Wffn1_packed) &&
+                CFM_ALIGNED16(b1f1) && CFM_ALIGNED16(colsum1) && CFM_ALIGNED16(b2_1) && CFM_ALIGNED16(Y) && CFM_ALIGNED16(Wqkv_packed) &&
+                CFM_ALIGNED16(bqkv) && CFM_ALIGNED16(csqkv) && CFM_ALIGNED16(Z), CFM_ERR_ALIGN);
+    if (M == 0) return CFM_OK;
+    ChainArgs a{C, ldc, Wpw2_packed, bpw2, R, ldr, nullptr, 0, nullptr, 0, ffn2_eps, Wffn2_packed, b1f2, colsum2, b2_2, alpha2, hidden,
+                cfm_ffn_tile_stride_f4(d), cfm_ffn_rotate(), Y, ldy, nullptr, gamma, beta, ln_eps, Wqkv_packed, bqkv, csqkv, att_eps, Z, ldz,
+                M, Wffn1_packed, b1f1, colsum1, b2_1, alpha1, ffn1_eps};
+    const dim3 grid((unsigned)((M + 31) / 32)), block(256);
+    hipStream_t s = static_cast<hipStream_t>(stream);
+    if (d == 512) hipLaunchKernelGGL((rowchain_f32_kernel<16, 1, 1, POST_BIAS3, CH_PLAIN, 1>), grid, block, 0, s, a);
+    else if (d == 256) hipLaunchKernelGGL((rowchain_f32_kernel<8, 1, 1, POST_BIAS3, CH_PLAIN, 1>), grid, block, 0, s, a);
+    else hipLaunchKernelGGL((rowchain_f32_kernel<4, 1, 1, POST_BIAS3, CH_PLAIN, 1>), grid, block, 0, s, a);
+    return cfm_launch_status();
+}
diff --git a/conformer_amd/model/modules/encoder.py b/conformer_amd/model/modules/encoder.py
--- a/conformer_amd/model/modules/encoder.py
+++ b/conformer_amd/model/modules/encoder.py
@@ -50,10 +50,30 @@
                 raise RuntimeError(f"lengths.max() after subsampling must equal T'={n_frames}")
         table = self.rel_pe.table(n_frames)
         pos_all = self._projected_positions(table)
+        if st is not None and self._seam_path(h):
+            return self._seam_layers(h, st, table, out_len, pos_all), out_len
         for i, layer in enumerate(self.layers):
             h, st = layer.fused_chain(h, table, out_len, None if pos_all is None else pos_all[:, i * d:(i + 1) * d],
                                       x_stats=st, want_stats=i + 1 < len(self.layers))
         return h, out_len
+
+    def _seam_path(self, h: torch.Tensor) -> bool:
+        d = h.shape[-1]
+        if ops.rowchain_ok(d, self.layers[0].ffn_1.hidden_linear.out_features, h.numel() // d):
+            return False
+        hid = self.layers[0].ffn_1.hidden_linear.out_features
+        return all(l.seam_ready(h) and l.ffn_1.hidden_linear.out_features == hid for l in self.layers)
+
+    def _seam_layers(self, h, st, table, out_len, pos_all):
+        d, n = h.shape[-1], len(self.layers)
+        y, qkv = self.layers[0].seam_head(h, st)
+        for i, layer in enumerate(self.layers):
+            c, y2 = layer.seam_middle(y, qkv, table, out_len, None if pos_all is None else pos_all[:, i * d:(i + 1) * d])
+            if i + 1 < n:
+                y, qkv = layer.seam_to(self.layers[i + 1], c, y2)
+            else:
+                h, _ = layer.seam_tail(c, y2)
+        return h
 
     def _projected_positions(self, table: torch.Tensor) -> Optional[torch.Tensor]:
         if len(self.layers) == 0:
diff --git a/conformer_amd/model/utils/block.py b/conformer_amd/model/utils/block.py
--- a/conformer_amd/model/utils/block.py
+++ b/conformer_amd/model/utils/block.py
@@ -94,6 +94,59 @@
         return ops.rowchain_pw2_ffn_ln(c, w2_p, pw2.bias, y2, ffn2, f2.out_linear.bias, 0.5, f2.layer_norm.eps,
                                        (ln.weight, ln.bias, ln.eps), want_stats)
 
+    def seam_ready(self, x: torch.Tensor) -> bool:
+        d = x.shape[-1]
+        h1, h2 = self.ffn_1.hidden_linear.out_features, self.ffn_2.hidden_linear.out_features
+        return bool(x.dim() == 3 and x.is_contiguous() and h1 == h2 and self._ln_fold(x)
+                    and ops.seam_chain_ok(d, h1, x.numel() // d))
+
+    def _seam_packs(self):
+        f1, f2, att, cv = self.ffn_1, self.ffn_2, self.attention, self.conv
+        a, ln_a = att.attention, att.layer_norm
+        for m, name in ((f1, "FeedForwardModule"), (att, "MultiHeadSelfAttentionModule"), (a, "RelativeMultiHeadAttention"),
+                        (cv, "ConvolutionModule"), (f2, "FeedForwardModule")):
+            refuse_dropout(m, name)
+        ffn1 = f1._packs.get("ffn_pack", (f1.hidden_linear.weight, f1.hidden_linear.bias, f1.layer_norm.weight, f1.layer_norm.bias,
+                                          f1.out_linear.weight), f1._pack)
+        ffn2 = f2._packs.get("ffn_pack", (f2.hidden_linear.weight, f2.hidden_linear.bias, f2.layer_norm.weight, f2.layer_norm.bias,
+                                          f2.out_linear.weight), f2._pack)
+        wqkv, bqkv = a._qkv_params()
+
+        def fold_pack():
+            wf, bf, cs = ops.fold_layernorm(wqkv, bqkv, ln_a.weight, ln_a.bias)
+            return ops.rowgemm_pack(wf), bf, cs
+
+        qkv = a._packs.get("qkv_chain", (wqkv, bqkv, ln_a.weight, ln_a.bias), fold_pack)
+        pw2 = cv.pointwise_conv_2
+        w2_p = cv._packs.get("pw2_chain", (pw2.weight,), lambda: ops.rowgemm_pack(pw2.weight.detach()))
+        return ffn1, ffn2, qkv, w2_p
+
+    def seam_head(self, x: torch.Tensor, x_stats: torch.Tensor):
+        ffn1, _, (wq_p, bq_f, csq), _ = self._seam_packs()
+        f1 = self.ffn_1
+        return ops.rowchain_ffn_qkv(x, x_stats, ffn1, f1.out_linear.bias, 0.5, f1.layer_norm.eps, wq_p, bq_f, csq,
+                                    self.attention.layer_norm.eps)
+
+    def seam_middle(self, y, qkv, pos_table, lengths, pos_projected):
+        a = self.attention.attention
+        pos = pos_projected if pos_projected is not None else ops.linear(pos_table, a.pos_proj.weight, a.pos_proj.bias)
+        ctx = ops.relpos_attention(qkv, pos, a.content_bias, a.position_bias, lengths, a.n_heads, for_gemm=True)
+        y2, st = ops.linear_residual(ctx, a.out_proj.weight, a.out_proj.bias, y, 1.0, emit_stats=True)
+        return self.conv.depthwise_lnfold(y2, st), y2
+
+    def seam_tail(self, c, y2, want_stats: bool = False):
+        _, ffn2, _, w2_p = self._seam_packs()
+        f2, ln, pw2 = self.ffn_2, self.layer_norm, self.conv.pointwise_conv_2
+        return ops.rowchain_pw2_ffn_ln(c, w2_p, pw2.bias, y2, ffn2, f2.out_linear.bias, 0.5, f2.layer_norm.eps,
+                                       (ln.weight, ln.bias, ln.eps), want_stats)
+
+    def seam_to(self, nxt: "ConformerBlock", c, y2):
+        _, ffn2, _, w2_p = self._seam_packs()
+        ffn1, _, (wq_p, bq_f, csq), _ = nxt._seam_packs()
+        f2, ln, pw2, f1 = self.ffn_2, self.layer_norm, self.conv.pointwise_conv_2, nxt.ffn_1
+        return ops.seam_chain(c, w2_p, pw2.bias, y2, ffn2, f2.out_linear.bias, 0.5, f2.layer_norm.eps, (ln.weight, ln.bias, ln.eps),
+                              ffn1, f1.out_linear.bias, 0.5, f1.layer_norm.eps, wq_p, bq_f, csq, nxt.attention.layer_norm.eps)
+
     def forward(self, x: torch.Tensor, pos_embedding: torch.Tensor, mask: Optional[torch.Tensor] = None) -> torch.Tensor:
         table = pos_embedding[0] if pos_embedding.dim() == 3 else pos_embedding
         lengths = None if mask is None else lengths_from_key_padding_mask(mask)
diff --git a/conformer_amd/model/utils/convolution.py b/conformer_amd/model/utils/convolution.py
--- a/conformer_amd/model/utils/convolution.py
+++ b/conformer_amd/model/utils/convolution.py
@@ -28,6 +28,16 @@
         bn = self.batch_norm
         return ops.dwconv_bn_swish(g, self.deepwise_conv.weight, self.deepwise_conv.bias, bn.weight, bn.bias,
                                    bn.running_mean, bn.running_var, bn.eps, for_gemm=for_gemm)
+
+    def depthwise_lnfold(self, x: torch.Tensor, stats: torch.Tensor, stream=None) -> torch.Tensor:
+        ln, pw1, dw, bn = self.layer_norm, self.pointwise_conv_1, self.deepwise_conv, self.batch_norm
+        wf, bf, cs = self._packs.get("ln_fold", (pw1.weight, pw1.bias, ln.weight, ln.bias),
+                                     lambda: ops.fold_layernorm(pw1.weight, pw1.bias, ln.weight, ln.bias))
+        if stream is None and x.dim() == 3 and ops.convmod_fused_ok(x.shape[0], x.shape[1], x.shape[2], dw.weight.shape[-1]):
+            return ops.convmod_glu_dwconv(x, stats, wf, bf, cs, ln.eps, dw.weight, dw.bias, bn.weight, bn.bias, bn.running_mean,
+                                          bn.running_var, bn.eps)
+        g = ops.linear_lnfold(x, stats, wf, bf, cs, ln.eps, glu=True)
+        return self.depthwise_eval(g, for_gemm=True) if stream is None else stream.depthwise(self, g)
 
     def fused(self, x: torch.Tensor, residual: Optional[torch.Tensor] = None, stats: Optional[torch.Tensor] = None,
               emit_stats: bool = False, stream=None):
@@ -61,20 +71,10 @@
                 bn.num_batches_tracked += 1
             return out if residual is not None else out - x
         if stats is not None:
-            ln, pw1 = self.layer_norm, self.pointwise_conv_1
-            wf, bf, cs = self._packs.get("ln_fold", (pw1.weight, pw1.bias, ln.weight, ln.bias),
-                                         lambda: ops.fold_layernorm(pw1.weight, pw1.bias, ln.weight, ln.bias))
-            dw = self.deepwise_conv
-            if stream is None and x.dim() == 3 and ops.convmod_fused_ok(x.shape[0], x.shape[1], x.shape[2], dw.weight.shape[-1]):
-                g = None
-                s = ops.convmod_glu_dwconv(x, stats, wf, bf, cs, ln.eps, dw.weight, dw.bias, bn.weight, bn.bias, bn.running_mean,
-                                           bn.running_var, bn.eps)
-            else:
-                g = ops.linear_lnfold(x, stats, wf, bf, cs, ln.eps, glu=True)
+            s = self.depthwise_lnfold(x, stats, stream)
         else:
             h = ops.layernorm(x, self.layer_norm.weight, self.layer_norm.bias, self.layer_norm.eps, for_gemm=stream is None)
             g = ops.linear_glu(h, self.pointwise_conv_1.weight, self.pointwise_conv_1.bias)
-        if g is not None:
             s = self.depthwise_eval(g, for_gemm=True) if stream is None else stream.depthwise(self, g)
         if residual is None:
             if emit_stats:
diff --git a/conformer_amd/ops.py b/conformer_amd/ops.py
--- a/conformer_amd/ops.py
+++ b/conformer_amd/ops.py
@@ -355,6 +355,48 @@
     _rowchain(1, 1, 0, 2, c, d, wpre=wpw2_p, bpre=_req(bpw2, "bias"), res=res, ln_eps=ffn_eps, ffn=ffn, b2=_req(b2, "b2"), alpha=alpha,
               y=out, stats_out=st, ln2=(_req(closing_ln[0], "ln.weight"), _req(closing_ln[1], "ln.bias"), float(closing_ln[2])))
     return out, st
+
+
+_SEAM_ENV = __import__("os").environ.get("CONFORMER_AMD_SEAM_CHAIN", "1")
+_SEAM_CHAIN = "force" if _SEAM_ENV == "force" else _SEAM_ENV != "0"
+
+
+def set_seam_chain(on):
+    global _SEAM_CHAIN
+    prev, _SEAM_CHAIN = _SEAM_CHAIN, ("force" if on == "force" else bool(on))
+    return prev
+
+
+def seam_chain_ok(d: int, hidden: int, rows: int) -> bool:
+    if not _SEAM_CHAIN:
+        return False
+    if _SEAM_CHAIN == "force":
+        return bool(ln_fold_ok(d) and d in (128, 256, 512) and hidden > 0 and hidden % 128 == 0 and rows > 0)
+    return ffn_fused_ok(d, hidden, rows)
+
+
+def seam_chain(c, wpw2_p, bpw2, res, ffn2, b2_2, alpha2: float, ffn2_eps: float, closing_ln, ffn1, b2_1, alpha1: float,
+               ffn1_eps: float, wqkv_p, bqkv_f, csqkv, att_eps: float):
+    c = _req(c, "c"); res = _req(res, "residual")
+    d = c.shape[-1]
+    rows = c.numel() // d
+    (wp2, b1f2, cs2), (wp1, b1f1, cs1) = ffn2, ffn1
+    hidden = b1f2.numel()
+    lib = _lib.load()
+    if b1f1.numel() != hidden or wp2.numel() != int(lib.cfm_ffn_pack_elems(d, hidden)) or wp1.numel() != wp2.numel() \
+            or tuple(res.shape) != tuple(c.shape) or wpw2_p.numel() != d * d or wqkv_p.numel() != 3 * d * d:
+        raise _lib.ConformerHipError(f"seam_chain: c{tuple(c.shape)}, residual{tuple(res.shape)}, hidden {hidden} / {b1f1.numel()} "
+                                     "and the packs do not match")
+    g2, bt2, eps2 = _req(closing_ln[0], "ln.weight"), _req(closing_ln[1], "ln.bias"), float(closing_ln[2])
+    y = torch.empty(c.shape, device=c.device, dtype=torch.float32)
+    qkv = torch.empty(*c.shape[:-1], 3 * d, device=c.device, dtype=torch.float32)
+    st = lib.cfm_seam_chain_f32(c.data_ptr(), d, wpw2_p.data_ptr(), _req(bpw2, "bias").data_ptr(), res.data_ptr(), d, float(ffn2_eps),
+                                wp2.data_ptr(), b1f2.data_ptr(), cs2.data_ptr(), _req(b2_2, "b2").data_ptr(), float(alpha2),
+                                g2.data_ptr(), bt2.data_ptr(), eps2, float(ffn1_eps), wp1.data_ptr(), b1f1.data_ptr(), cs1.data_ptr(),
+                                _req(b2_1, "b2").data_ptr(), float(alpha1), hidden, y.data_ptr(), d, wqkv_p.data_ptr(),
+                                bqkv_f.data_ptr(), csqkv.data_ptr(), float(att_eps), qkv.data_ptr(), 3 * d, rows, d, _stream())
+    _lib.check(st, "cfm_seam_chain_f32")
+    return y, qkv
 
 
 def layernorm(x: torch.Tensor, weight: torch.Tensor, bias: torch.Tensor, eps: float = 1e-5,
diff --git a/include/conformer_hip.h b/include/conformer_hip.h
--- a/include/conformer_hip.h
+++ b/include/conformer_hip.h
@@ -71,6 +71,12 @@
                      const float* b2, float alpha, int hidden, float* Y, int64_t ldy, float* stats_out,
                      const float* gamma2, const float* beta2, float eps2, const float* Wpost_packed, const float* bpost,
                      const float* cspost, float post_eps, float* Z, int64_t ldz, int64_t M, int d, cfm_stream_t stream);
+int cfm_seam_chain_f32(const float* C, int64_t ldc, const float* Wpw2_packed, const float* bpw2, const float* R, int64_t ldr,
+                       float ffn2_eps, const float* Wffn2_packed, const float* b1f2, const float* colsum2, const float* b2_2,
+                       float alpha2, const float* gamma, const float* beta, float ln_eps, float ffn1_eps,
+                       const float* Wffn1_packed, const float* b1f1, const float* colsum1, const float* b2_1, float alpha1,
+                       int hidden, float* Y, int64_t ldy, const float* Wqkv_packed, const float* bqkv, const float* csqkv,
+                       float att_eps, float* Z, int64_t ldz, int64_t M, int d, cfm_stream_t stream);
 int64_t cfm_ffn_tile_stride_f4(int d);
 int cfm_ffn_rotate(void);
 
```

After: 1.733 million audio-frames/sec, median of 6. No clear change (+0.8%).
